# computational-cell-analytics/micro-sam

Measured on AMD Instinct MI355X. Metric: 1024^2 tiles/s embed+AMG (vit_b bf16), higher is better.
Workload: dtype bf16 image encoder (patch embedding + neck, 1.2 % of its flops, on hi+lo operand pairs of that type), fp16 mask decoder (16-bit MFMA operands, fp32 accumulation); 1 GPU; configs[1]: vit_b, 1024x1024 uint8 synthetic tiles, batched embedding precompute + AutomaticMaskGenerator (32x32 grid, multimask, default thresholds); encoder_batch=16, distinct_tiles_per_gpu=256, weights=seeded synthetic checkpoint (synthetic.py variant 'cells'), decode_lanes=3

## Files before the change

### include/msam_hip.h

```cpp
#ifndef MSAM_HIP_H
#define MSAM_HIP_H

#include <stdint.h>

#ifdef __cplusplus
extern "C" {
#endif

#define MSAM_MAX_BLOCKS 32
#define MSAM_F32 1
#define MSAM_BF16 2
#define MSAM_FP8 3
#define MSAM_F16 4
#define MSAM_U8 5
#define MSAM_U16 6
#define MSAM_ACT_NONE 0
#define MSAM_ACT_GELU 1
#define MSAM_ACT_RELU 2
#define MSAM_ACT_SIGMOID 3

const char* msam_last_error(void);
int msam_abi_version(void);


// ... 2 lines not shown
    const void* W; int64_t ldw;
    int32_t M, N, K;
    const float* bias;
    const float* table;
    int32_t table_rows, table_cols;
    int64_t table_ld;
    const void* resid;
    int32_t resid_dtype; int32_t resid_rows;
    int64_t ldr;
    int32_t act;
    void* out; int32_t out_dtype; int64_t ldc;
    int32_t out_mode;
    void* q; void* k; void* v;
    int32_t heads, head_dim, tokens;
    int32_t use_glds;
    int32_t ln_mode;
    const float* ln_w; const float* ln_b; float ln_eps;
    int32_t a_dtype;
    const float* row_scale; const float* col_scale;
    int32_t split_k;
    const float* ln_add; void* ln_out_a; void* ln_out_b;
} msam_gemm_t;
int msam_gemm_bf16(const msam_gemm_t* p, void* stream);
#define MSAM_GEMM_GROUP_MAX 5
int msam_gemm_group_bf16(const msam_gemm_t* items, int32_t n, void* stream);

typedef struct {
    const void* A; const void* W; int32_t M, N, K;
    const float* bias;
    const float* table; int32_t table_rows, table_cols; int64_t table_ld;
    const void* resid; int32_t resid_rows; int64_t ldr;
    int32_t ln_mode; const float* ln_w; const float* ln_b; float ln_eps;
    void* out; int64_t ldc;
    int32_t kv_split; void* k_out; void* vT_out; int32_t tokens;
    int32_t head_major;
} msam_wsgemm_t;
int msam_wsgemm_bf16(const msam_wsgemm_t* p, void* stream);

typedef struct {
    const void* xin; const void* q_shared;
    const void* wq; const float* bq; const float* peq;
    const void* wo; const float* bo; const float* ln_w; const float* ln_b; float ln_eps;
    const void* ktok; const void* vtok; int32_t Nt;
    void* out; int32_t rows;
} msam_image_layer_t;
int msam_decoder_image_layer(const msam_image_layer_t* p, void* stream);

int64_t msam_t2i_fold_workspace_bytes(int32_t P);
int msam_t2i_fold_attention(const void* keys, int32_t kv_shared, const void* qtok, int32_t P, int32_t Nt, const void* wk,
                            const void* tabk, const void* wv, const float* bv, void* out, void* workspace,
                            int64_t workspace_bytes, void* stream);

int64_t msam_i2t_fold_workspace_bytes(int32_t P);
int msam_i2t_fold_layer(const void* xin, int32_t x_shared, const void* ktok, const void* vtok, int32_t P, int32_t Nt,
                        const void* wq, const void* tabq, const void* wo, const float* bo, const float* ln_w,
                        const float* ln_b, float ln_eps, void* out, void* workspace, int64_t workspace_bytes, void* stream);

int64_t msam_chain_tables_bytes(void);
int msam_chain_prepare_tables(const void* src, const void* q0, const void* tabk, const void* tabq1, void* tables, void* stream);
int64_t msam_i2t_fold_operand_bytes(int32_t P);
int msam_i2t_fold_operands(const void* ktok, const void* vtok, int32_t P, int32_t Nt, const void* wq, const void* wo,
                           const float* bo, int32_t with_kfold, void* operands, void* stream);
int64_t msam_i2t0_t2i_workspace_bytes(int32_t P);
int msam_i2t0_t2i_fused(const void* tables, const void* operands0, const float* ln0_w, const float* ln0_b, float ln_eps,
                        const void* qtok, int32_t P, int32_t Nt, const void* wk, const void* wv, const float* bv, void* out,
                        void* workspace, int64_t workspace_bytes, void* stream);
int64_t msam_chain_tables2_bytes(void);
int msam_chain_prepare_tables2(const void* src, const void* wv, const float* bv, const void* wk, const float* ln0_w,
                               const float* ln0_b, const void* wo0, const float* bo0, void* tables2, void* stream);
int64_t msam_chain_const2_bytes(void);
int msam_chain_prepare_const2(const void* wv, const float* bv, const void* wk, const float* ln0_w, const float* ln0_b,
                              const void* wo0, const float* bo0, void* const2, void* stream);
int msam_chain_prepare_tables2_c(const void* src, const void* const2, void* tables2, void* stream);
int64_t msam_t2i_fold_values_bytes(int32_t P);
int msam_t2i_fold_values(const void* vtok0, int32_t P, int32_t Nt, const void* tables2, void* mf, void* stream);
int msam_i2t_fold_operands_values(const void* ktok, const void* vtok, int32_t P, int32_t Nt, const void* wq, const void* wo,
                                  const float* bo, int32_t with_kfold, const void* tables2, void* operands, void* mf, void* stream);
int64_t msam_i2t0_t2i_v2_workspace_bytes(int32_t P);
int msam_i2t0_t2i_fused_v2(const void* tables, const void* tables2, const void* operands0, const void* mf, const float* ln0_w,
                           float ln_eps, const void* qtok, int32_t P, int32_t Nt, const void* wk, void* out, void* workspace,
                           int64_t workspace_bytes, void* stream);
int msam_i2t01_fused(const void* tables, const void* operands0, const float* ln0_w, const float* ln0_b, const void* operands1,
                     const float* ln1_w, const float* ln1_b, float ln_eps, int32_t P, int32_t Nt, void* out, void* stream);

int msam_upscale_fused(const void* keys, int32_t P, const void* w1, const float* b1, const float* ln_w, const float* ln_b,
                       float ln_eps, const void* w2, const float* b2, const float* hyper, int32_t hyper_ld, int32_t mask0,
                       int32_t nmask, float* low_res, void* stream);
int msam_upscale_fused_layout(const void* keys, int32_t keys_blocked, int32_t P, const void* w1, const float* b1,
                              const float* ln_w, const float* ln_b, float ln_eps, const void* w2, const float* b2,
                              const float* hyper, int32_t hyper_ld, int32_t mask0, int32_t nmask, float* low_res, void* stream);
int msam_upscale_fused_out(const void* keys, int32_t keys_blocked, int32_t P, const void* w1, const float* b1,
                           const float* ln_w, const float* ln_b, float ln_eps, const void* w2, const float* b2,
                           const float* hyper, int32_t hyper_ld, int32_t mask0, int32_t nmask, void* low_res,
                           int32_t low_res_dtype, void* stream);

int msam_upscale_set_prio(int32_t prio);
int msam_fold_attn_set_dma(int32_t on);
int msam_tune_set(const char* key, int32_t value);
int msam_debug_i2t_timing(int32_t enable, uint64_t* host_out);
int msam_gemm256_set_staging(int staging);
int msam_gemm_set_trace(void* device_words);
int msam_profile_enable(int on);
int msam_profile_collect(int32_t* launches, double* total_ms, double* total_flops);
#define MSAM_PROFILE_FAMILIES 8
int msam_profile_collect_family(int32_t* launches, double* ms, double* flops, double* bytes);

int msam_to_image(const void* in, int32_t in_dtype, int32_t H, int32_t W, int32_t C, uint8_t* out, void* workspace, void* stream);

int msam_mask_nms(const uint32_t* bits, const int32_t* order, const float* boxes, const int32_t* area, int32_t K, int32_t H,
                  int32_t W, float thresh, int32_t intersection_over_min, uint64_t* mask_scratch, int32_t* keep_flags,
                  void* stream);

int64_t msam_amg_generate_workspace_bytes(int32_t N, int32_t H, int32_t W);
int msam_amg_generate_labels(const float* iou, const float* stability, const int32_t* boxes, const int32_t* area,
                             const uint32_t* bits, int32_t N, int32_t H, int32_t W, const int32_t* crop_box,
                             float pred_iou_thresh, float stability_score_thresh, float box_nms_thresh,
                             int32_t min_object_size, int32_t with_background, int32_t* labels, int32_t* flag,
                             void* workspace, int64_t workspace_bytes, void* stream);

int64_t msam_labels_from_masks_workspace_bytes(int32_t H, int32_t W);
int msam_labels_from_masks(const uint32_t* bits, const int32_t* order, int32_t K, const int32_t* k_dev, int32_t H, int32_t W,
                           int32_t min_object_size, int32_t with_background, int32_t* labels, int32_t* flag,
                           void* workspace, int64_t workspace_bytes, void* stream);

int msam_layernorm_backward(const float* x, const float* weight, const float* dy, float eps, int64_t rows, int32_t dim,
                            float* dx, float* dweight, float* dbias, void* stream);
int msam_attention_forward(const float* q, const float* k, const float* v, int32_t BH, int32_t Nq, int32_t Nk, int32_t D,
                           float scale, float* out, float* lse, void* stream);
int msam_attention_backward(const float* q, const float* k, const float* v, const float* out, const float* dout,
                            const float* lse, int32_t BH, int32_t Nq, int32_t Nk, int32_t D, float scale, float* dq, float* dk,
                            float* dv, float* delta, void* stream);

int msam_relpos_attention_forward(const float* q, const float* k, const float* v, const float* bias_h, const float* bias_w,
                                  int32_t BH, int32_t Gh, int32_t Gw, int32_t D, float scale, float* out, float* lse,
                                  void* stream);
int msam_relpos_attention_backward(const float* q, const float* k, const float* v, const float* bias_h, const float* bias_w,
                                   const float* out, const float* dout, const float* lse, int32_t BH, int32_t Gh, int32_t Gw,
                                   int32_t D, float scale, float* dq, float* dk, float* dv, float* dbias_h, float* dbias_w,
                                   float* delta, void* stream);

int msam_cast_transpose(const void* x, int32_t x_dtype, int64_t M, int32_t K, int64_t ldx, void* out16, void* outT, float* colsum,
                        void* stream);

int msam_layernorm(const float* x, const float* weight, const float* bias, float eps, int64_t rows, int32_t dim,
                   void* out, int32_t out_dtype, int32_t gelu, int32_t out_nchw_hw, void* stream);

int msam_layernorm_fp8(const float* x, const float* weight, const float* bias, float eps, int64_t rows, int32_t dim,
                       void* out_fp8, float* row_scale, void* stream);
int msam_quant_rows_fp8(const void* x_bf16, int64_t rows, int32_t dim, void* out_fp8, float* row_scale, void* stream);
int msam_patchify(const float* img, int32_t B, void* out_bf16, void* stream);
int msam_patchify16(const float* img, int32_t B, int32_t dtype16, void* out16, void* stream);
int msam_patchify_u8(const uint8_t* img, int32_t B, int32_t h, int32_t w, void* out_bf16, void* stream);
int msam_patchify_u8_16(const uint8_t* img, int32_t B, int32_t h, int32_t w, int32_t dtype16, void* out16, void* stream);
int msam_im2col3x3(const void* x_bf16, int32_t B, int32_t C, void* out_bf16, void* stream);
int msam_cast_f32_to_bf16(const float* x, void* out_bf16, int64_t n, void* stream);
int msam_cast_f32_to_16(const float* x, int32_t dtype16, void* out16, int64_t n, void* stream);
int msam_resample_u8(const uint8_t* in, int32_t B, int32_t H, int32_t W, int32_t C, int32_t axis, int32_t n_out,
                     const int32_t* bounds, const int32_t* coefs, int32_t ksize, uint8_t* out, void* stream);
int msam_patchify_split16(const float* img, int32_t B, int32_t dtype16, void* out16, void* stream);
int msam_patchify_u8_split16(const uint8_t* img, int32_t B, int32_t h, int32_t w, int32_t dtype16, void* out16, void* stream);
int msam_im2col3x3_split16(const float* x_f32, int32_t B, int32_t C, int32_t dtype16, void* out16, void* stream);
int msam_cast_f32_split16(const float* x, int32_t dtype16, void* out16, int64_t rows, int32_t dim, void* stream);

int msam_window_attention(const void* q, const void* k, const void* v, const void* rel_h, const void* rel_w,
                          const float* qkv_bias, int32_t B, int32_t heads, int32_t head_dim, float scale, void* out,
                          void* stream);
// ... 274 lines not shown
```

### micro_sam_amd/_lib.py

```python
from __future__ import annotations

import ctypes as C
import os
from typing import Optional

import torch

from . import build as _build

MSAM_MAX_BLOCKS = 32
F32, BF16, FP8, F16, U8, U16 = 1, 2, 3, 4, 5, 6
ACT_NONE, ACT_GELU, ACT_RELU, ACT_SIGMOID = 0, 1, 2, 3

_vp, _i32, _i64, _f32 = C.c_void_p, C.c_int32, C.c_int64, C.c_float
PROFILE_FAMILIES = 8


class GemmParams(C.Structure):
    _fields_ = [
        ("A", _vp), ("lda", _i64), ("W", _vp), ("ldw", _i64), ("M", _i32), ("N", _i32), ("K", _i32),
        ("bias", _vp), ("table", _vp), ("table_rows", _i32), ("table_cols", _i32), ("table_ld", _i64),
        ("resid", _vp), ("resid_dtype", _i32), ("resid_rows", _i32), ("ldr", _i64), ("act", _i32),
        ("out", _vp), ("out_dtype", _i32), ("ldc", _i64), ("out_mode", _i32),
        ("q", _vp), ("k", _vp), ("v", _vp), ("heads", _i32), ("head_dim", _i32), ("tokens", _i32),
# ... 63 lines not shown


class SGemmParams(C.Structure):
    _fields_ = [("A", _vp), ("lda", _i64), ("A2", _vp), ("lda2", _i64), ("a2_rows", _i64), ("W", _vp), ("ldw", _i64),
                ("M", _i64), ("N", _i32), ("K", _i32), ("bias", _vp), ("act", _i32), ("res", _vp), ("ldr", _i64), ("res_rows", _i64),
                ("out", _vp), ("ldc", _i64), ("col_scale", _vp), ("col_shift", _vp), ("conv_h", _i32), ("conv_w", _i32), ("conv_c", _i32),
                ("shuffle_h", _i32), ("shuffle_w", _i32), ("shuffle_c", _i32), ("a2_cols", _i32), ("split16", _i32), ("a_scale", _f32), ("w_scale", _f32), ("w_pairs", _vp)]


class SI2TParams(C.Structure):
    _fields_ = [("keys", _vp), ("key_batch_stride", _i64), ("pos", _vp), ("wq", _vp), ("bq", _vp), ("tok_k", _vp), ("tok_v", _vp),
                ("ld_tok", _i64), ("tok_batch_stride", _i64), ("wo", _vp), ("bo", _vp), ("ln_weight", _vp), ("ln_bias", _vp),
                ("ln_eps", _f32), ("denom", _f32), ("out", _vp), ("B", _i32), ("Tk", _i32), ("split16", _i32), ("wq_scale", _f32), ("wo_scale", _f32), ("wq_pairs", _vp), ("wo_pairs", _vp)]


class ST2IParams(C.Structure):
    _fields_ = [("keys", _vp), ("key_batch_stride", _i64), ("pos", _vp), ("q", _vp), ("ldq", _i64), ("wk", _vp), ("wv", _vp), ("bv", _vp),
                ("denom", _f32), ("out", _vp), ("ldo", _i64), ("B", _i32), ("Tk", _i32), ("workspace", _vp), ("workspace_bytes", _i64)]


class SUp2Params(C.Structure):
    _fields_ = [("u1", _vp), ("ln_weight", _vp), ("ln_bias", _vp), ("ln_eps", _f32), ("w2", _vp), ("b2", _vp), ("w_scale", _f32),
                ("hyper", _vp), ("hyper_ld", _i32), ("mask0", _i32), ("nmask", _i32), ("low_res", _vp), ("P", _i64)]


class MaskPromptParams(C.Structure):
    _fields_ = [(n, _vp) for n in ("c1_w", "c1_b", "ln1_w", "ln1_b", "c2_w", "c2_b", "ln2_w", "ln2_b", "c3_w", "c3_b")] + [("exact_gelu", _i32)]


_PROTOS = {
    "msam_last_error": (C.c_char_p, []),
    "msam_abi_version": (_i32, []),
    "msam_gemm_bf16": (_i32, [C.POINTER(GemmParams), _vp]),
    "msam_wsgemm_bf16": (_i32, [C.POINTER(WsGemmParams), _vp]),
    "msam_decoder_image_layer": (_i32, [C.POINTER(ImageLayerParams), _vp]),
    "msam_t2i_fold_workspace_bytes": (_i64, [_i32]),
    "msam_t2i_fold_attention": (_i32, [_vp, _i32, _vp, _i32, _i32, _vp, _vp, _vp, _vp, _vp, _vp, _i64, _vp]),
    "msam_upscale_fused": (_i32, [_vp, _i32, _vp, _vp, _vp, _vp, _f32, _vp, _vp, _vp, _i32, _i32, _i32, _vp, _vp]),
    "msam_uncrop_bits": (_i32, [_vp, _i32, _i32, _i32, _i32, _i32, _i32, _i32, _vp, _vp]),
    "msam_decoder_forward_masks": (_i32, [C.POINTER(DecoderParams), C.POINTER(MaskPromptParams), _vp, _vp, _vp, _vp, _i32, _vp, _vp,
                                          _i32, _i32, _vp, _vp, _vp, _i64, _vp]),
    "msam_i2t_fold_workspace_bytes": (_i64, [_i32]),
    "msam_i2t_fold_layer": (_i32, [_vp, _i32, _vp, _vp, _i32, _i32, _vp, _vp, _vp, _vp, _vp, _vp, _f32, _vp, _vp, _i64, _vp]),
    "msam_profile_enable": (_i32, [_i32]),
    "msam_profile_collect": (_i32, [C.POINTER(_i32), C.POINTER(C.c_double), C.POINTER(C.c_double)]),
    "msam_profile_collect_family": (_i32, [_i32 * PROFILE_FAMILIES, C.c_double * PROFILE_FAMILIES, C.c_double * PROFILE_FAMILIES,
                                          C.c_double * PROFILE_FAMILIES]),
    "msam_layernorm": (_i32, [_vp, _vp, _vp, _f32, _i64, _i32, _vp, _i32, _i32, _i32, _vp]),
    "msam_layernorm_backward": (_i32, [_vp, _vp, _vp, _f32, _i64, _i32, _vp, _vp, _vp, _vp]),
    "msam_attention_forward": (_i32, [_vp, _vp, _vp, _i32, _i32, _i32, _i32, _f32, _vp, _vp, _vp]),
    "msam_attention_backward": (_i32, [_vp, _vp, _vp, _vp, _vp, _vp, _i32, _i32, _i32, _i32, _f32, _vp, _vp, _vp, _vp, _vp]),
    "msam_relpos_attention_forward": (_i32, [_vp, _vp, _vp, _vp, _vp, _i32, _i32, _i32, _i32, _f32, _vp, _vp, _vp]),
    "msam_relpos_attention_backward": (_i32, [_vp, _vp, _vp, _vp, _vp, _vp, _vp, _vp, _i32, _i32, _i32, _i32, _f32, _vp, _vp, _vp,
                                              _vp, _vp, _vp, _vp]),
    "msam_amg_generate_workspace_bytes": (_i64, [_i32, _i32, _i32]),
    "msam_amg_generate_labels": (_i32, [_vp, _vp, _vp, _vp, _vp, _i32, _i32, _i32, C.POINTER(_i32), _f32, _f32, _f32, _i32, _i32,
                                        _vp, _vp, _vp, _i64, _vp]),
    "msam_to_image": (_i32, [_vp, _i32, _i32, _i32, _i32, _vp, _vp, _vp]),
    "msam_patchify": (_i32, [_vp, _i32, _vp, _vp]),
    "msam_patchify_u8": (_i32, [_vp, _i32, _i32, _i32, _vp, _vp]),
    "msam_im2col3x3": (_i32, [_vp, _i32, _i32, _vp, _vp]),
    "msam_cast_f32_to_bf16": (_i32, [_vp, _vp, _i64, _vp]),
    "msam_cast_transpose": (_i32, [_vp, _i32, _i64, _i32, _i64, _vp, _vp, _vp, _vp]),
    "msam_gemm256_set_staging": (_i32, [_i32]),
    "msam_gemm_set_trace": (_i32, [_vp]),
    "msam_gemm_group_bf16": (_i32, [_vp, _i32, _vp]),
    "msam_fold_attn_set_dma": (_i32, [_i32]),
    "msam_tune_set": (_i32, [C.c_char_p, _i32]),
    "msam_i2t_fold_operand_bytes": (_i64, [_i32]),
    "msam_i2t_fold_operands": (_i32, [_vp, _vp, _i32, _i32, _vp, _vp, _vp, _i32, _vp, _vp]),
    "msam_i2t0_t2i_workspace_bytes": (_i64, [_i32]),
    "msam_i2t0_t2i_fused": (_i32, [_vp, _vp, _vp, _vp, _f32, _vp, _i32, _i32, _vp, _vp, _vp, _vp, _vp, _i64, _vp]),
    "msam_i2t01_fused": (_i32, [_vp, _vp, _vp, _vp, _vp, _vp, _vp, _f32, _i32, _i32, _vp, _vp]),
    "msam_chain_tables2_bytes": (_i64, []),
    "msam_chain_prepare_tables2": (_i32, [_vp, _vp, _vp, _vp, _vp, _vp, _vp, _vp, _vp, _vp]),
    "msam_chain_const2_bytes": (_i64, []),
    "msam_chain_prepare_const2": (_i32, [_vp, _vp, _vp, _vp, _vp, _vp, _vp, _vp, _vp]),
    "msam_chain_prepare_tables2_c": (_i32, [_vp, _vp, _vp, _vp]),
    "msam_t2i_fold_values_bytes": (_i64, [_i32]),
    "msam_t2i_fold_values": (_i32, [_vp, _i32, _i32, _vp, _vp, _vp]),
    "msam_i2t_fold_operands_values": (_i32, [_vp, _vp, _i32, _i32, _vp, _vp, _vp, _i32, _vp, _vp, _vp, _vp]),
    "msam_i2t0_t2i_v2_workspace_bytes": (_i64, [_i32]),
    "msam_i2t0_t2i_fused_v2": (_i32, [_vp, _vp, _vp, _vp, _vp, _f32, _vp, _i32, _i32, _vp, _vp, _vp, _i64, _vp]),
    "msam_chain_tables_bytes": (_i64, []),
    "msam_chain_prepare_tables": (_i32, [_vp, _vp, _vp, _vp, _vp, _vp]),
    "msam_upscale_fused_layout": (_i32, [_vp, _i32, _i32, _vp, _vp, _vp, _vp, _f32, _vp, _vp, _vp, _i32, _i32, _i32, _vp, _vp]),
    "msam_upscale_fused_out": (_i32, [_vp, _i32, _i32, _vp, _vp, _vp, _vp, _f32, _vp, _vp, _vp, _i32, _i32, _i32, _vp, _i32, _vp]),
    "msam_upscale_set_prio": (_i32, [_i32]),
    "msam_layernorm_fp8": (_i32, [_vp, _vp, _vp, _f32, _i64, _i32, _vp, _vp, _vp]),
    "msam_quant_rows_fp8": (_i32, [_vp, _i64, _i32, _vp, _vp, _vp]),
    "msam_debug_i2t_timing": (_i32, [_i32, _vp]),
    "msam_window_attention": (_i32, [_vp, _vp, _vp, _vp, _vp, _vp, _i32, _i32, _i32, C.c_float, _vp, _vp]),
    "msam_global_attention": (_i32, [_vp, _vp, _vp, _vp, _vp, _i32, _i32, _i32, C.c_float, _vp, _vp]),
    "msam_window_attention16": (_i32, [_vp, _vp, _vp, _vp, _vp, _vp, _i32, _i32, _i32, C.c_float, _i32, _vp, _vp]),
    "msam_global_attention16": (_i32, [_vp, _vp, _vp, _vp, _vp, _i32, _i32, _i32, C.c_float, _i32, _vp, _vp]),
    "msam_patchify16": (_i32, [_vp, _i32, _i32, _vp, _vp]),
    "msam_patchify_u8_16": (_i32, [_vp, _i32, _i32, _i32, _i32, _vp, _vp]),
    "msam_cast_f32_to_16": (_i32, [_vp, _i32, _vp, _i64, _vp]),
    "msam_resample_u8": (_i32, [_vp, _i32, _i32, _i32, _i32, _i32, _i32, _vp, _vp, _i32, _vp, _vp]),
    "msam_patchify_split16": (_i32, [_vp, _i32, _i32, _vp, _vp]),
    "msam_patchify_u8_split16": (_i32, [_vp, _i32, _i32, _i32, _i32, _vp, _vp]),
    "msam_im2col3x3_split16": (_i32, [_vp, _i32, _i32, _i32, _vp, _vp]),
    "msam_cast_f32_split16": (_i32, [_vp, _i32, _vp, _i64, _i32, _vp]),
    "msam_encoder_workspace_bytes": (_i64, [C.POINTER(EncoderParams), _i32]),
    "msam_encoder_forward": (_i32, [C.POINTER(EncoderParams), _vp, _vp, _i32, _i32, _i32, _vp, _vp, _i64, _vp, _i32, _vp]),
    "msam_decoder_dtype": (_i32, []),
    "msam_decoder_const_bytes": (_i64, []),
    "msam_decoder_prepare_const": (_i32, [C.POINTER(DecoderParams), _vp, _vp]),
    "msam_decoder_image_bytes": (_i64, []),
    "msam_decoder_prepare_image": (_i32, [C.POINTER(DecoderParams), _vp, _vp, _vp, _vp, _i64, _vp]),
    "msam_decoder_workspace_bytes": (_i64, [_i32]),
    "msam_prompt_encode": (_i32, [C.POINTER(DecoderParams), C.POINTER(MaskPromptParams), _vp, _vp, _i32, _vp, _vp, _i32, _vp, _vp, _vp]),
    "msam_decoder_forward_embeddings": (_i32, [C.POINTER(DecoderParams), _vp, _vp, _vp, _i32, _vp, _vp, _i32, _i32, _vp, _vp, _vp,
                                               _i64, _vp]),
    "msam_decoder_forward": (_i32, [C.POINTER(DecoderParams), _vp, _vp, _vp, _vp, _i32, _vp, _i32, _i32, _vp, _vp, _vp,
                                    _i64, _vp]),
    "msam_postprocess_masks": (_i32, [_vp, _i32, _i32, _i32, _i32, _i32, _f32, _f32, _vp, _vp, _vp, _vp, _vp]),
    "msam_postprocess_masks16": (_i32, [_vp, _i32, _i32, _i32, _i32, _i32, _i32, _f32, _f32, _vp, _vp, _vp, _vp, _vp]),
    "msam_rle_run_counts": (_i32, [_vp, _i32, _i32, _i32, _vp, _vp]),
    "msam_rle_encode": (_i32, [_vp, _i32, _i32, _i32, _vp, _vp, _vp]),
    "msam_mask_nms": (_i32, [_vp, _vp, _vp, _vp, _i32, _i32, _i32, _f32, _i32, _vp, _vp, _vp]),
    "msam_box_nms": (_i32, [_vp, _i32, _f32, _vp, _vp, _vp]),
    "msam_box_nms_valid": (_i32, [_vp, _vp, _i32, _f32, _vp, _vp, _vp]),
    "msam_paint_label_image_dev": (_i32, [_vp, _vp, _vp, _i32, _i32, _vp, _vp]),
    "msam_label_components_async": (_i32, [_vp, _i32, _i32, _vp, _vp, _i32, _vp]),
    "msam_component_sizes": (_i32, [_vp, _i32, _vp, _vp, _vp]),
    "msam_labels_from_masks_workspace_bytes": (_i64, [_i32, _i32]),
    "msam_labels_from_masks": (_i32, [_vp, _vp, _i32, _vp, _i32, _i32, _i32, _i32, _vp, _vp, _vp, _i64, _vp]),
    "msam_host_seeded_watershed": (_i32, [_vp, _vp, _vp, _i32, _i32, _vp]),
    "msam_slice_overlaps": (_i32, [_vp, _i32, _i32, _i32, _vp, _vp, _i32, _vp, _i32, _vp, _vp]),
    "msam_paint_label_image": (_i32, [_vp, _vp, _i32, _i32, _i32, _vp, _vp]),
    "msam_label_components": (_i32, [_vp, _i32, _i32, _vp, _vp, _i32, C.POINTER(_i32), _vp]),
    "msam_strict_gemm": (_i32, [C.POINTER(SGemmParams), _vp]),
    "msam_strict_i2t_block": (_i32, [C.POINTER(SI2TParams), _vp]),
    "msam_strict_layernorm": (_i32, [_vp, _vp, _vp, _f32, _i64, _i32, _vp, _i32, _i32, _vp]),
    "msam_strict_relpos_attention": (_i32, [_vp, _vp, _vp, _vp, _i32, _i32, _i32, _i32, _i32, _f32, _vp, _vp]),
    "msam_split16_relpos_attention": (_i32, [_vp, _vp, _vp, _vp, _i32, _i32, _i32, _i32, _i32, _f32, _vp, _vp]),
    "msam_strict_attention": (_i32, [_vp, _i64, _i64, _vp, _i64, _i64, _vp, _i64, _i64, _i32, _i32, _i32, _i32, _i32, _f32, _vp, _i64,
                                     _i64, _vp]),
    "msam_strict_patchify": (_i32, [_vp, _vp, _i32, _i32, _i32, _vp, _vp]),
    "msam_strict_im2col3x3": (_i32, [_vp, _i32, _i32, _vp, _vp]),
    "msam_strict_source": (_i32, [_vp, _vp, _i64, _i32, _vp, _vp]),
    "msam_strict_hyper_masks": (_i32, [_vp, _vp, _i32, _i32, _i32, _i64, _vp, _vp]),
    "msam_strict_upscale2": (_i32, [C.POINTER(SUp2Params), _vp]),
    "msam_split16_t2i_attention": (_i32, [C.POINTER(ST2IParams), _vp]),
    "msam_split16_prepare_pairs": (_i32, [_vp, _i64, _i32, _f32, _i32, _vp, _vp]),
    "msam_split16_i2t_block": (_i32, [C.POINTER(SI2TParams), _vp, _i64, _vp]),
    "msam_strict_instance_norm": (_i32, [_vp, _i64, _i32, _i64, _i32, _f32, _vp, _vp, _i64, _vp]),
    "msam_strict_resize_bilinear": (_i32, [_vp, _i32, _i32, _i32, _i32, _i32, _i64, _i32, _i32, _i32, _f32, _f32, _i32, _vp, _vp]),
    "msam_objfeat_gather": (_i32, [_vp, _vp, _i32, _i32, _vp, _vp, _i32, _vp, _vp, _vp]),
    "msam_objfeat_accumulate": (_i32, [_vp, _vp, _i32, _vp, _vp, _vp, _vp, _vp, _vp, _vp, _i32, _i32, _i32, _vp, _vp]),
    "msam_objfeat_finish": (_i32, [_vp, _vp, _vp, _i32, _vp, _vp, _i32, _vp, _vp]),
    "msam_objfeat_project": (_i32, [_vp, _i64, _vp, _i32, _vp, _vp]),
    "msam_label_matching_workspace_bytes": (_i64, [_i32, _i32]),
    "msam_label_matching": (_i32, [_vp, _vp, _i32, _i32, _i32, _i32, C.POINTER(C.c_double), _i32, _vp, _i64, _i32, _vp, _i32, _vp]),
    "msam_edt_squared_workspace_bytes": (_i64, [_i32, _i32]),
    "msam_edt_squared": (_i32, [_vp, _i32, _i32, _i32, _vp, _vp, _i64, _vp]),
    "msam_label_props_workspace_bytes": (_i64, [_i32, _i32, _i32]),
    "msam_label_props": (_i32, [_vp, _i32, _i32, _vp, _i32, _vp, _vp, _vp, _vp, _vp, _i64, _vp]),
    "msam_distance_targets_workspace_bytes": (_i64, [_i32, _i32, _i32]),
    "msam_distance_targets": (_i32, [_vp, _i32, _i32, _i32, _i32, _f32, _vp, _vp, _vp, _vp, _vp, _i64, _vp]),
    "msam_mask_pack": (_i32, [_vp, _i32, _i32, _i32, _vp, _vp]),
    "msam_mask_iou_counts": (_i32, [_vp, _vp, _i32, _i32, _i32, C.c_double, _vp, _vp, _vp]),
    "msam_mask_box_prompts": (_i32, [_vp, _i32, _i32, _i32, C.c_double, _i32, _i32, _vp, _vp, _vp]),
    "msam_mask_logits": (_i32, [_vp, _i32, _i32, _i32, _vp, _vp]),
    "msam_paint_max": (_i32, [_vp, _vp, _vp, _i32, _i32, _i32, _vp, _vp]),
# ... 78 lines not shown
```

### micro_sam_amd/csrc/decfold.hip

```cpp
#include "common.h"
#include "../../include/msam_hip.h"
#include <string>

void msam_set_error(const char* msg);
int msam_check_launch(const char* what);
void msam_profile_mark2(void* stream, int begin, double flops, double bytes, int family);

namespace {

constexpr int T = 4096, C = 256, CI = 128, TK = 32, NTHR = 256;
constexpr int SUBT = 1024 + 32;
constexpr int KEYS_BYTES = 16 * SUBT, TAB_BYTES = TK * CI * 2, BUF_BYTES = KEYS_BYTES + TAB_BYTES;
constexpr float NEG_BIG = -1.0e30f;
#ifndef FOLD_ATTN_DMA_DEFAULT
#define FOLD_ATTN_DMA_DEFAULT 0
#endif

typedef short s16x4_t __attribute__((ext_vector_type(4)));

MSAM_DEVINL uint2 lds_tr16(const unsigned char* p) {
    s16x4_t v = __builtin_amdgcn_ds_read_tr16_b64_v4i16((s16x4_t __attribute__((address_space(3)))*)p);
    return __builtin_bit_cast(uint2, v);
}

// ... 594 lines not shown
    const double bytes = (double)((kv_shared & 1) ? 1 : P) * T * C * 2 + (KS > 1 ? (double)P * KS * 64 * C * 4 : 0.0);
    msam_profile_mark2(stream, 1, flops, bytes, 3);
    if (g_fold_attn_dma && !a.blocked) {
        const int grid3 = a.nitems < 3 * cus ? a.nitems : 3 * cus;
        hipLaunchKernelGGL(fold_attn_kernel<true>, dim3(grid3), dim3(NTHR), 0, s, a);
    } else {
        hipLaunchKernelGGL(fold_attn_kernel<false>, dim3(grid), dim3(NTHR), 0, s, a);
    }
    msam_profile_mark2(stream, 0, flops, bytes, 3);
    if (int e = msam_check_launch("fold_attn")) return e;
    if (KS == 1) return 0;
    hipLaunchKernelGGL(fold_finish_kernel, dim3(P * 8), dim3(128), 0, s, opart, stats, KS, Nt, (const u16*)wv, bv, (u16*)out);
    return msam_check_launch("fold_finish");
}

int64_t msam_i2t_tok_workspace_bytes(int32_t P);
int msam_i2t_tok_layer(const void* xin, int32_t x_shared, const void* ktok, const void* vtok, int32_t P, int32_t Nt,
                       const void* wq, const void* tabq, const void* wo, const float* bo, const float* ln_w,
                       const float* ln_b, float ln_eps, void* out, void* workspace, int KS, void* stream);
extern int g_tune_i2t_variant;

extern "C" int64_t msam_i2t_fold_workspace_bytes(int32_t P) {
    const int64_t a = (int64_t)P * 64 * C * 2 * 2, b = msam_i2t_tok_workspace_bytes(P);
    return a > b ? a : b;
}

extern "C" int msam_i2t_fold_layer(const void* xin, int32_t x_shared, const void* ktok, const void* vtok, int32_t P,
                                   int32_t Nt, const void* wq, const void* tabq, const void* wo, const float* bo,
                                   const float* ln_w, const float* ln_b, float ln_eps, void* out, void* workspace,
                                   int64_t workspace_bytes, void* stream) {
    if (!xin || !ktok || !vtok || !wq || !tabq || !wo || !bo || !ln_w || !ln_b || !out || !workspace || P <= 0) {
        msam_set_error("msam_i2t_fold_layer: null argument");
        return 1;
    }
    if (Nt < 1 || Nt > 8) { msam_set_error("msam_i2t_fold_layer: 1 <= Nt <= 8 tokens per prompt"); return 1; }
    if (workspace_bytes < msam_i2t_fold_workspace_bytes(P)) { msam_set_error("msam_i2t_fold_layer: workspace too small"); return 1; }
    if (g_tune_i2t_variant == 1)
        return msam_i2t_tok_layer(xin, x_shared, ktok, vtok, P, Nt, wq, tabq, wo, bo, ln_w, ln_b, ln_eps, out, workspace,
                                  key_splits(P), stream);
    hipStream_t s = (hipStream_t)stream;
    u16* kfold = (u16*)workspace;
    u16* vfoldT = kfold + (long)P * 64 * C;
    hipLaunchKernelGGL(fold_q_kernel, dim3(P * 8), dim3(256), 0, s, (const u16*)ktok, (const u16*)wq, Nt, kfold);
    if (int e = msam_check_launch("fold_k")) return e;
    hipLaunchKernelGGL(fold_v_kernel, dim3(P), dim3(256), 0, s, (const u16*)vtok, (const u16*)wo, Nt, vfoldT);
    if (int e = msam_check_launch("fold_v")) return e;
    I2tArgs a{};
    a.xin = (const u16*)xin; a.x_shared = x_shared; a.kfold = kfold; a.vfoldT = vfoldT; a.ktok = (const u16*)ktok; a.Nt = Nt;
    a.tabq = (const u16*)tabq; a.bo = bo; a.ln_w = ln_w; a.ln_b = ln_b; a.eps = ln_eps;
    a.KS = key_splits(P); a.nitems = P * a.KS; a.out = (u16*)out;
    int dev = 0, cus = 256;
    (void)hipGetDevice(&dev);
    (void)hipDeviceGetAttribute(&cus, hipDeviceAttributeMultiprocessorCount, dev);
    const int grid = a.nitems < 2 * cus ? a.nitems : 2 * cus;
    const double flops = (double)P * T * (2.0 * 64 * C * 2 + 2.0 * 64 * 32);
    const double bytes = (double)(x_shared ? 1 : P) * T * C * 2 + (double)P * T * C * 2;
    msam_profile_mark2(stream, 1, flops, bytes, 2);
    if (g_i2t_timing) hipLaunchKernelGGL(fold_i2t_kernel<true>, dim3(grid), dim3(NTHR), 0, s, a);
    else hipLaunchKernelGGL(fold_i2t_kernel<false>, dim3(grid), dim3(NTHR), 0, s, a);
    msam_profile_mark2(stream, 0, flops, bytes, 2);
    return msam_check_launch("fold_i2t");
}

extern "C" int msam_debug_i2t_timing(int32_t enable, uint64_t* host_out) {
    g_i2t_timing = enable;
    if (host_out) {
        if (hipDeviceSynchronize() != hipSuccess ||
            hipMemcpyFromSymbol(host_out, HIP_SYMBOL(g_i2t_stamps), sizeof(unsigned long long) * 64 * 12) != hipSuccess) {
            msam_set_error("msam_debug_i2t_timing: copy failed");
            return 2;
        }
    }
    return 0;
}

extern "C" int msam_fold_attn_set_dma(int32_t on) { g_fold_attn_dma = on; return 0; }

extern int g_tune_i2t_wg_per_cu, g_tune_chain_variant, g_tune_chain_tmask, g_tune_up_gelu16, g_tune_up_ln_two_pass, g_tune_up_centred;
void msam_gemm_set_dbg(int v);
void msam_gemm_set_gw(int delay, int cls);
void msam_gemm_set_g3(int delay);
void msam_gemm_set_g3_epi(int v);
extern int g_tune_tok_fuse;
extern int g_tune_mlp_split_fused;
extern int g_tune_sgemm_bufs, g_tune_srel_mfma, g_tune_sgemm_small_below, g_tune_si2t_dbg, g_tune_si2t_late_us, g_tune_sattn_allh;
int g_tune_dec_chain = 1, g_tune_dec_chain_min_p = 128;
extern "C" int msam_tune_set(const char* key, int32_t value) {
    const std::string k = key ? key : "";
    if (k == "i2t_variant") g_tune_i2t_variant = value;
    else if (k == "i2t_wg_per_cu") g_tune_i2t_wg_per_cu = value;
    else if (k == "dec_chain") g_tune_dec_chain = value;
    else if (k == "chain_variant") g_tune_chain_variant = value;
    else if (k == "chain_tmask") g_tune_chain_tmask = value;
    else if (k == "up_gelu16") g_tune_up_gelu16 = value;
    else if (k == "up_ln_two_pass") g_tune_up_ln_two_pass = value;
    else if (k == "up_centred") g_tune_up_centred = value;
    else if (k == "gemm_dbg") msam_gemm_set_dbg(value);
    else if (k == "gw_delay") msam_gemm_set_gw(value, -1);
    else if (k == "gw_class") msam_gemm_set_gw(-2, value);
    else if (k == "g3_delay") msam_gemm_set_g3(value);
    else if (k == "g3_epi") msam_gemm_set_g3_epi(value);
    else if (k == "tok_fuse") g_tune_tok_fuse = value;
    else if (k == "mlp_split_fused") g_tune_mlp_split_fused = value;
    else if (k == "dec_chain_min_p") g_tune_dec_chain_min_p = value;
    else if (k == "sgemm_bufs") g_tune_sgemm_bufs = value;
    else if (k == "srel_mfma") g_tune_srel_mfma = value;
    else if (k == "sattn_allh") g_tune_sattn_allh = value;
    else if (k == "sgemm_small_below") g_tune_sgemm_small_below = value;
    else if (k == "si2t_dbg") g_tune_si2t_dbg = value;
    else if (k == "si2t_late_us") g_tune_si2t_late_us = value;
    else { msam_set_error("msam_tune_set: unknown key"); return 1; }
    return 0;
}
```

### micro_sam_amd/csrc/decfold_tok.hip

```cpp
#include "common.h"
#include "../../include/msam_hip.h"

void msam_set_error(const char* msg);
int msam_check_launch(const char* what);
void msam_profile_mark2(void* stream, int begin, double flops, double bytes, int family);

int g_tune_i2t_variant = 1;
int g_tune_i2t_wg_per_cu = 2;
int g_tune_chain_tmask = 255;
int g_tune_chain_variant = 9;

namespace {

constexpr int T = 4096, C = 256, CI = 128, NTHR = 256;
constexpr int FRAG = 1024;
constexpr int KT_OFF = 0, KT_BYTES = 4 * 2 * FRAG;
constexpr int KF_OFF = KT_OFF + KT_BYTES, KF_BYTES = 4 * 8 * FRAG;
constexpr int VF_OFF = KF_OFF + KF_BYTES, VF_BYTES = 2 * 16 * FRAG;
constexpr int OPER_BYTES = VF_OFF + VF_BYTES;
constexpr float NEG_BIG = -1.0e30f;
constexpr float SCALE = 0.25f * 1.4426950408889634f;

__global__ __launch_bounds__(256) void fold_frag_kernel(const u16* __restrict__ ktok, const u16* __restrict__ vtok,
                                                        const u16* __restrict__ wq, const u16* __restrict__ wo,
                                                        const float* __restrict__ bo, int Nt, int with_kf,
                                                        u16* __restrict__ oper, const unsigned char* __restrict__ t2 = nullptr,
                                                        u16* __restrict__ mf = nullptr) {
    __shared__ __attribute__((aligned(16))) u16 img[OPER_BYTES / 2];
    __shared__ float kk[8][CI], vv[8][CI];
    const int p = blockIdx.x, c = threadIdx.x;
    for (int i = c; i < 8 * CI; i += 256) {
        const int t = i >> 7, d = i & (CI - 1);
        kk[t][d] = t < Nt ? d2f(ktok[((long)p * Nt + t) * CI + d]) : 0.f;
        vv[t][d] = t < Nt ? d2f(vtok[((long)p * Nt + t) * CI + d]) : 0.f;
    }
    for (int i = c; i < KT_BYTES / 16; i += 256) ((uint4*)img)[KT_OFF / 16 + i] = make_uint4(0, 0, 0, 0);
    __syncthreads();
    if (with_kf) {
        const int ks = c >> 5, fg = (c >> 3) & 3, ii = c & 7;
        for (int h = 0; h < 8; ++h) {
            float w[16];
#pragma unroll
            for (int d = 0; d < 16; ++d) w[d] = d2f(wq[(h * 16 + d) * C + c]);
#pragma unroll
            for (int t = 0; t < 8; ++t) {
                float acc = 0.f;
#pragma unroll
                for (int d = 0; d < 16; ++d) acc = fmaf(kk[t][h * 16 + d], w[d], acc);
                const int m = 2 * (h >> 2) + (t >> 2), fr = 4 * (h & 3) + (t & 3);
                img[KF_OFF / 2 + ((m * 8 + ks) * 64 + fg * 16 + fr) * 8 + ii] = f2d(acc * SCALE);
            }
        }
    }
    for (int j = c; j < 8 * 8 * 16; j += 256) {
        const int h = j >> 7, t = (j >> 4) & 7, d = j & 15;
        const int m = 2 * (h >> 2) + (t >> 2), e = (h >> 1) & 1, fr = 4 * (h & 3) + (t & 3), fg = 2 * (h & 1) + (d >> 3);
        img[KT_OFF / 2 + ((m * 2 + e) * 64 + fg * 16 + fr) * 8 + (d & 7)] = f2d(kk[t][h * 16 + d] * SCALE);
    }
    {
        const int cp = c >> 5, within = c & 31, rho = 4 * (within >> 3) + (within & 3), ct = 2 * cp + ((within >> 2) & 1);
        const float bo8 = bo[c] * 0.125f;
        for (int h = 0; h < 8; ++h) {
            const uint4 w0 = *(const uint4*)(wo + (long)c * CI + h * 16), w1 = *(const uint4*)(wo + (long)c * CI + h * 16 + 8);
            const uint32_t ww[8] = {w0.x, w0.y, w0.z, w0.w, w1.x, w1.y, w1.z, w1.w};
            float wf[16];
#pragma unroll
            for (int x = 0; x < 8; ++x) { wf[2 * x] = d2f((u16)(ww[x] & 0xffff)); wf[2 * x + 1] = d2f((u16)(ww[x] >> 16)); }
            uint32_t pk[4];
#pragma unroll
            for (int t2 = 0; t2 < 4; ++t2) {
                float a0 = 0.f, a1 = 0.f;
#pragma unroll
                for (int d = 0; d < 16; ++d) { a0 = fmaf(wf[d], vv[2 * t2][h * 16 + d], a0); a1 = fmaf(wf[d], vv[2 * t2 + 1][h * 16 + d], a1); }
                pk[t2] = pack2d(2 * t2 < Nt ? a0 + bo8 : 0.f, 2 * t2 + 1 < Nt ? a1 + bo8 : 0.f);
            }
            const int a = h >> 2, fg = h & 3;
            *(uint4*)(img + VF_OFF / 2 + ((a * 16 + ct) * 64 + fg * 16 + rho) * 8) = make_uint4(pk[0], pk[1], pk[2], pk[3]);
        }
    }
    if (t2) {
        const int d = c & 127, hh = c >> 7;
        const float* wowv = (const float*)t2 + d * 128;
        const float cd8 = ((const float*)(t2 + 128 * 128 * 4))[d] * 0.125f;
        u16* mdst = mf + (long)p * (16 * FRAG / 2);
        for (int h = hh * 4; h < hh * 4 + 4; ++h) {
            float wv_[16];
#pragma unroll
            for (int e = 0; e < 16; ++e) wv_[e] = wowv[h * 16 + e];
            uint32_t pk[4];
#pragma unroll
            for (int t2_ = 0; t2_ < 4; ++t2_) {
                float a0 = 0.f, a1 = 0.f;
#pragma unroll
// ... 93 lines not shown
    const float nmr = -mean * rstd;
#pragma unroll
    for (int c2 = 0; c2 < 8; ++c2) {
        const float4 g0 = *(const float4*)(gp + c2 * 32), g1 = *(const float4*)(gp + c2 * 32 + 4);
        const float4 h0 = *(const float4*)(gp + C + c2 * 32), h1 = *(const float4*)(gp + C + c2 * 32 + 4);
        const f32x4_t x0 = o[2 * c2], x1 = o[2 * c2 + 1];
        y[c2].x = pack2d(fmaf(fmaf(x0[0], rstd, nmr), g0.x, h0.x), fmaf(fmaf(x0[1], rstd, nmr), g0.y, h0.y));
        y[c2].y = pack2d(fmaf(fmaf(x0[2], rstd, nmr), g0.z, h0.z), fmaf(fmaf(x0[3], rstd, nmr), g0.w, h0.w));
        y[c2].z = pack2d(fmaf(fmaf(x1[0], rstd, nmr), g1.x, h1.x), fmaf(fmaf(x1[1], rstd, nmr), g1.y, h1.y));
        y[c2].w = pack2d(fmaf(fmaf(x1[2], rstd, nmr), g1.z, h1.z), fmaf(fmaf(x1[3], rstd, nmr), g1.w, h1.w));
    }
}

struct TokArgs {
    const u16* xin; int x_shared;
    const u16* oper;
    const u16* tabq;
    const float* ln_w; const float* ln_b; float eps;
    int Nt, nitems, KS;
    u16* out;
};

__global__ __launch_bounds__(NTHR, 2) void i2t_tok_kernel(TokArgs a) {
    __shared__ __attribute__((aligned(16))) unsigned char lds[OPER_BYTES + 2 * C * 4];
    const int tid = threadIdx.x, lane = tid & 63, w = __builtin_amdgcn_readfirstlane(tid >> 6), fr = lane & 15, fg = lane >> 4;
    const int ks_sh = __builtin_ctz(a.KS), tpi_sh = 8 - ks_sh;
    const int TPI = 1 << tpi_sh, nt = TPI >> 2;
    float* prm = (float*)(lds + OPER_BYTES);
    prm[tid] = a.ln_w[tid]; prm[C + tid] = a.ln_b[tid];
    const WaveConst wc = wave_const(fr, fg, a.Nt);
    const int voff = fr * (C * 2) + fg * 16;
    const int tvoff = fr * (CI * 2) + fg * 16;
    const rsrc_t rtab = make_rsrc(a.tabq, T * CI * 2);
    const unsigned char* const L = lds + lane * 16;
    const float* const gp = prm + fg * 8;

    for (int item = (int)blockIdx.x; item < a.nitems; item += (int)gridDim.x) {
        const int p = __builtin_amdgcn_readfirstlane(item >> ks_sh), split = __builtin_amdgcn_readfirstlane(item & (a.KS - 1));
        __syncthreads();
        {
            const uint4* src = (const uint4*)(a.oper + (long)p * (OPER_BYTES / 2));
#pragma unroll 6
            for (int i = tid; i < OPER_BYTES / 16; i += NTHR) ((uint4*)lds)[i] = src[i];
        }
        __syncthreads();
        const rsrc_t rx = make_rsrc(a.xin + (long)(a.x_shared ? 0 : p) * T * C, T * C * 2);
        const rsrc_t ro = make_rsrc(a.out + (long)p * T * C, T * C * 2);
        const int tile0 = split * TPI + w;

        uint4 b[8], tb[4];
#define TK_LOAD(tile_)                                                                             \
        do {                                                                                       \
            const int so_ = (tile_) * (16 * C * 2), to_ = (tile_) * (16 * CI * 2);                 \
            _Pragma("unroll") for (int s_ = 0; s_ < 8; ++s_) b[s_] = buf_load16(rx, voff, so_ + s_ * 64);      \
            _Pragma("unroll") for (int s_ = 0; s_ < 4; ++s_) tb[s_] = buf_load16(rtab, tvoff, to_ + s_ * 64);  \
        } while (0)
        TK_LOAD(tile0);
        wait_vmem_all();
        for (int n = 0; n < nt; ++n) {
            asm volatile("" ::: "memory");
            const int tile = tile0 + 4 * n;
            uint4 y[8];
            i2t_block<KT_OFF, KF_OFF, VF_OFF, true>(L, gp, a.eps, b, tb, wc, y, [&]() {
                const int nx = tile0 + 4 * (n + 1 < nt ? n + 1 : nt - 1);
                TK_LOAD(nx);
            });
#pragma unroll
            for (int c2 = 0; c2 < 8; ++c2) buf_store16(y[c2], ro, voff, tile * (16 * C * 2) + c2 * 64);
        }
#undef TK_LOAD
    }
}

struct ChainArgs {
    const u16* src;
    const u16* q0;
    const u16* oper0;
    const float* ln0_w; const float* ln0_b;
    const u16* oper1;
    const u16* tabq1;
    const float* ln1_w; const float* ln1_b;
    float eps; int Nt, P;
    u16* out;
};

constexpr int NTHR8 = 512;
constexpr int C_KT0 = 0, C_VF0 = C_KT0 + KT_BYTES, C_KT1 = C_VF0 + VF_BYTES, C_KF1 = C_KT1 + KT_BYTES, C_VF1 = C_KF1 + KF_BYTES,
              C_PRM = C_VF1 + VF_BYTES, C_LDS = C_PRM + 4 * C * 4;

__global__ __launch_bounds__(NTHR8, 2) void i2t01_kernel(ChainArgs a) {
    __shared__ __attribute__((aligned(16))) unsigned char lds[C_LDS];
    const int tid = threadIdx.x, lane = tid & 63, w = __builtin_amdgcn_readfirstlane(tid >> 6), fr = lane & 15, fg = lane >> 4;
    float* prm = (float*)(lds + C_PRM);
    if (tid < C) { prm[tid] = a.ln0_w[tid]; prm[C + tid] = a.ln0_b[tid]; }
    else { prm[2 * C + tid - C] = a.ln1_w[tid - C]; prm[3 * C + tid - C] = a.ln1_b[tid - C]; }
    const WaveConst wc = wave_const(fr, fg, a.Nt);
    const int voff = lane * 16, tvoff = lane * 16;
    const rsrc_t rsrc = make_rsrc(a.src, T * C * 2), rq0 = make_rsrc(a.q0, T * CI * 2), rtab = make_rsrc(a.tabq1, T * CI * 2);
    const unsigned char* const L = lds + lane * 16;
    const float* const gp0 = prm + fg * 8;
    const float* const gp1 = prm + 2 * C + fg * 8;
    constexpr int NT = 256 / 8;

    for (int p = (int)blockIdx.x; p < a.P; p += (int)gridDim.x) {
        __syncthreads();
        {
            const uint4* s0 = (const uint4*)(a.oper0 + (long)p * (OPER_BYTES / 2));
            const uint4* s1 = (const uint4*)(a.oper1 + (long)p * (OPER_BYTES / 2));
            for (int i = tid; i < KT_BYTES / 16; i += NTHR8) ((uint4*)(lds + C_KT0))[i] = s0[KT_OFF / 16 + i];
            for (int i = tid; i < VF_BYTES / 16; i += NTHR8) ((uint4*)(lds + C_VF0))[i] = s0[VF_OFF / 16 + i];
#pragma unroll 3
            for (int i = tid; i < OPER_BYTES / 16; i += NTHR8) ((uint4*)(lds + C_KT1))[i] = s1[i];
        }
        __syncthreads();
        const rsrc_t ro = make_rsrc(a.out + (long)p * T * C, T * C * 2);
        uint4 b[8], qi[4], tb[4];
#define CH_LOAD0(tile_)                                                                            \
        do {                                                                                       \
            const int so_ = (tile_) * (16 * C * 2), to_ = (tile_) * (16 * CI * 2);                 \
            _Pragma("unroll") for (int s_ = 0; s_ < 8; ++s_) b[s_] = buf_load16(rsrc, voff, so_ + s_ * FRAG);    \
            _Pragma("unroll") for (int s_ = 0; s_ < 4; ++s_) qi[s_] = buf_load16(rq0, tvoff, to_ + s_ * FRAG);   \
        } while (0)
#define CH_LOAD1(tile_)                                                                            \
        do {                                                                                       \
            const int to_ = (tile_) * (16 * CI * 2);                                               \
            _Pragma("unroll") for (int s_ = 0; s_ < 4; ++s_) tb[s_] = buf_load16(rtab, tvoff, to_ + s_ * FRAG);  \
        } while (0)
        CH_LOAD0(w); CH_LOAD1(w);
        wait_vmem_all();
        for (int n = 0; n < NT; ++n) {
            asm volatile("" ::: "memory");
            const int tile = w + 8 * n, nx = w + 8 * (n + 1 < NT ? n + 1 : NT - 1);
            uint4 y1[8], y2[8];
            i2t_block<C_KT0, 0, C_VF0, false>(L, gp0, a.eps, b, qi, wc, y1, [&]() { CH_LOAD0(nx); });
            i2t_block<C_KT1, C_KF1, C_VF1, true>(L, gp1, a.eps, y1, tb, wc, y2, [&]() { CH_LOAD1(nx); });
#pragma unroll
            for (int c2 = 0; c2 < 8; ++c2) buf_store16(y2[c2], ro, voff, tile * (16 * C * 2) + c2 * FRAG);
        }
#undef CH_LOAD0
#undef CH_LOAD1
    }
}

struct AttnState { f32x4_t o[8]; float m[4], l[4]; };

template <int QD, int QF, int WV, class F>
MSAM_DEVINL void t2i_block(const unsigned char* L, const uint4* y, const uint4* tk, AttnState& st, F&& consumed) {
    f32x4_t s[4];
    uint4 fa[4], fb[4];
#pragma unroll
    for (int ct = 0; ct < 4; ++ct) s[ct] = f32x4_t{0.f, 0.f, 0.f, 0.f};
    TK_RD4(fa, QF, 8 * FRAG);
    TK_FENCE();
#pragma unroll
    for (int g = 0; g < 9; ++g) {
        uint4* cur = (g & 1) ? fb : fa;
        uint4* nxt = (g & 1) ? fa : fb;
        if (g + 1 < 8) TK_RD4(nxt, QF + (g + 1) * FRAG, 8 * FRAG);
        else if (g + 1 < 9) TK_RD4(nxt, QD, FRAG);
        else TK_RD4(nxt, WV, 8 * FRAG);
#pragma unroll
        for (int ct = 0; ct < 4; ++ct) s[ct] = mfma16d(g < 8 ? y[g < 8 ? g : 0] : tk[ct], cur[ct], s[ct]);
        TK_FENCE();
    }
    consumed();
    float mloc[4];
    bool need = false;
// ... 72 lines not shown
    float* prm = (float*)(lds + F_PRM);
    if (tid < C) prm[tid] = a.ln0_w[tid]; else prm[tid] = a.ln0_b[tid - C];
    for (int i = tid; i < WV_BYTES / 16; i += NTHR8) ((uint4*)(lds + F_WV))[i] = ((const uint4*)a.wvfrag)[i];
    const WaveConst wc = wave_const(fr, fg, a.Nt);
    const int voff = lane * 16, tvoff = lane * 16;
    const rsrc_t rsrc = make_rsrc(a.src, T * C * 2), rq0 = make_rsrc(a.q0, T * CI * 2), rtab = make_rsrc(a.tabk, T * CI * 2);
    const unsigned char* const L = lds + lane * 16;
    const float* const gp0 = prm + fg * 8;
    constexpr int NT = 256 / 8;

    for (int p = (int)blockIdx.x; p < a.P; p += (int)gridDim.x) {
        __syncthreads();
        {
            const uint4* s0 = (const uint4*)(a.oper0 + (long)p * (OPER_BYTES / 2));
            const uint4* s1 = (const uint4*)(a.aoper + (long)p * (AOPER_BYTES / 2));
            for (int i = tid; i < KT_BYTES / 16; i += NTHR8) ((uint4*)(lds + F_KT0))[i] = s0[KT_OFF / 16 + i];
            for (int i = tid; i < VF_BYTES / 16; i += NTHR8) ((uint4*)(lds + F_VF0))[i] = s0[VF_OFF / 16 + i];
            for (int i = tid; i < AOPER_BYTES / 16; i += NTHR8) ((uint4*)(lds + F_QD))[i] = s1[i];
        }
        __syncthreads();
        AttnState st;
#pragma unroll
        for (int h = 0; h < 8; ++h) st.o[h] = f32x4_t{0.f, 0.f, 0.f, 0.f};
#pragma unroll
        for (int ct = 0; ct < 4; ++ct) { st.m[ct] = NEG_BIG; st.l[ct] = 0.f; }
        uint4 b[8], qi[4], tk[4];
#define FU_LOAD0(tile_)                                                                            \
        do {                                                                                       \
            const int so_ = (tile_) * (16 * C * 2), to_ = (tile_) * (16 * CI * 2);                 \
            _Pragma("unroll") for (int s_ = 0; s_ < 8; ++s_) b[s_] = buf_load16(rsrc, voff, so_ + s_ * FRAG);    \
            _Pragma("unroll") for (int s_ = 0; s_ < 4; ++s_) qi[s_] = buf_load16(rq0, tvoff, to_ + s_ * FRAG);   \
        } while (0)
#define FU_LOAD1(tile_)                                                                            \
        do {                                                                                       \
            const int to_ = (tile_) * (16 * CI * 2);                                               \
            _Pragma("unroll") for (int s_ = 0; s_ < 4; ++s_) tk[s_] = buf_load16(rtab, tvoff, to_ + s_ * FRAG);  \
        } while (0)
        FU_LOAD0(w); FU_LOAD1(w);
        for (int n = 0; n < NT; ++n) {
            asm volatile("" ::: "memory");
            const int nx = w + 8 * (n + 1 < NT ? n + 1 : NT - 1);
            uint4 y1[8];
            i2t_block<F_KT0, 0, F_VF0, false>(L, gp0, a.eps, b, qi, wc, y1, [&]() { FU_LOAD0(nx); });
            t2i_block<F_QD, F_QF, F_WV>(L, y1, tk, st, [&]() { FU_LOAD1(nx); });
        }
#undef FU_LOAD0
#undef FU_LOAD1
#pragma unroll
        for (int ct = 0; ct < 4; ++ct) { st.l[ct] += __shfl_xor(st.l[ct], 16); st.l[ct] += __shfl_xor(st.l[ct], 32); }
        __syncthreads();
        float* mg = (float*)lds + w * MERGE_FLOATS;
        if (fg == 0) {
#pragma unroll
            for (int ct = 0; ct < 4; ++ct) { mg[ct * 16 + fr] = st.m[ct]; mg[64 + ct * 16 + fr] = st.l[ct]; }
        }
#pragma unroll
        for (int h = 0; h < 8; ++h)
            if ((fr >> 3) == (h & 1))
                *(float4*)(mg + 128 + (h * 8 + (fr & 7)) * 16 + fg * 4) = make_float4(st.o[h][0], st.o[h][1], st.o[h][2], st.o[h][3]);
        __syncthreads();
        {
            const int col = tid >> 3, d0 = (tid & 7) * 2, h = col >> 3, t = col & 7;
            const float* g0 = (const float*)lds;
            float mx = NEG_BIG;
#pragma unroll
            for (int ww = 0; ww < 8; ++ww) mx = fmaxf(mx, g0[ww * MERGE_FLOATS + col]);
            float lt = 0.f, o0 = 0.f, o1 = 0.f;
#pragma unroll
            for (int ww = 0; ww < 8; ++ww) {
                const float* gw = g0 + ww * MERGE_FLOATS;
                const float sc = __builtin_amdgcn_exp2f(gw[col] - mx);
                lt = fmaf(sc, gw[64 + col], lt);
                o0 = fmaf(sc, gw[128 + col * 16 + d0], o0); o1 = fmaf(sc, gw[128 + col * 16 + d0 + 1], o1);
            }
            if (t < a.Nt) {
                const float inv = 1.f / lt;
                *(uint32_t*)(a.out + ((long)p * a.Nt + t) * CI + h * 16 + d0) =
                    pack2d(fmaf(o0, inv, a.bv[h * 16 + d0]), fmaf(o1, inv, a.bv[h * 16 + d0 + 1]));
            }
        }
    }
}

template <int G, int D = 2> struct Ring { uint4 buf[D][G]; };

template <int G, class Off, int ABL = 0>
MSAM_DEVINL void ring_fill(Ring<G, Off::D>& r, const unsigned char* L, int batch) {
    if (ABL & 32) return;
#pragma unroll
    for (int j = 0; j < G; ++j) r.buf[batch % Off::D][j] = *(const uint4*)(L + Off::off((batch * G + j) % Off::N));
}
#define RING_STEP(n_) do { if ((n_) % G == 0) { TK_FENCE(); ring_fill<G, Off, ABL>(ring, L, (n_) / G + Off::D - 1); TK_FENCE(); } } while (0)
#define RING_AT(n_) ring.buf[((n_) / G) % Off::D][(n_) % G]

template <int G, class Off, int BASE, bool HAS_KF, int ABL = 0, bool AFFINE = true, class F>
MSAM_DEVINL void i2t_block_r(Ring<G, Off::D>& ring, const unsigned char* L, const float* gp, float eps, const uint4* b, const uint4* tb,
                             const WaveConst& wc, uint4* y, F&& consumed, uint4* pk_out = nullptr, float* stat_out = nullptr) {
    constexpr int NS = HAS_KF ? 40 : 8, G0 = HAS_KF ? 0 : 8;
    f32x4_t s[4];
#pragma unroll
    for (int m = 0; m < 4; ++m) s[m] = wc.sinit[m & 1];
#pragma unroll
    for (int i = 0; i < NS; ++i) {
        const int n = BASE + i, g = G0 + i / 4, m = i % 4;
        RING_STEP(n);
        if (!(ABL & 1)) s[m] = mfma16d(RING_AT(n), g < 8 ? b[g < 8 ? g : 0] : tb[2 * (m >> 1) + (g < 8 ? 0 : g - 8)], s[m]);
        else if (i < 4) s[m][0] += __uint_as_float((RING_AT(n).x ^ tb[m].x) & 0x3fffffffu);
    }
    f32x4_t o[16];
#pragma unroll
    for (int ct = 0; ct < 16; ++ct) o[ct] = mfma16d(wc.sel[ct & 1], b[ct >> 1], f32x4_t{0.f, 0.f, 0.f, 0.f});
    consumed();
    uint4 pk[2];
#pragma unroll
    for (int a2 = 0; a2 < 2; ++a2) {
        const f32x4_t u = s[2 * a2], v = s[2 * a2 + 1];
        const float mx = fmaxf(fmaxf(fmaxf(u[0], u[1]), fmaxf(u[2], u[3])), fmaxf(fmaxf(v[0], v[1]), fmaxf(v[2], v[3])));
        float eu[4], ev[4];
#pragma unroll
        for (int r = 0; r < 4; ++r) {
            eu[r] = (ABL & 64) ? u[r] - mx : __builtin_amdgcn_exp2f(u[r] - mx); ev[r] = (ABL & 64) ? v[r] - mx : __builtin_amdgcn_exp2f(v[r] - mx);
        }
        const float l = ((eu[0] + eu[1]) + (eu[2] + eu[3])) + ((ev[0] + ev[1]) + (ev[2] + ev[3]));
        const float inv = __builtin_amdgcn_rcpf(l);
        pk[a2] = make_uint4(pack2d(eu[0] * inv, eu[1] * inv), pack2d(eu[2] * inv, eu[3] * inv),
                            pack2d(ev[0] * inv, ev[1] * inv), pack2d(ev[2] * inv, ev[3] * inv));
    }
#pragma unroll
    for (int i = 0; i < 32; ++i) {
        const int n = BASE + NS + i;
        RING_STEP(n);
        if (!(ABL & 2) || i % 16 == 0) o[i % 16] = mfma16d(RING_AT(n), pk[i / 16], o[i % 16]);
    }
    if (ABL & 4) {
#pragma unroll
        for (int c2 = 0; c2 < 8; ++c2)
            y[c2] = make_uint4(pack2d(o[2 * c2][0], o[2 * c2][1]), pack2d(o[2 * c2][2], o[2 * c2][3]),
                               pack2d(o[2 * c2 + 1][0], o[2 * c2 + 1][1]), pack2d(o[2 * c2 + 1][2], o[2 * c2 + 1][3]));
        return;
    }
    float s1 = 0.f, s2 = 0.f;
#pragma unroll
    for (int ct = 0; ct < 16; ++ct)
#pragma unroll
        for (int r = 0; r < 4; ++r) { s1 += o[ct][r]; s2 = fmaf(o[ct][r], o[ct][r], s2); }
    s1 += __shfl_xor(s1, 16); s2 += __shfl_xor(s2, 16);
    s1 += __shfl_xor(s1, 32); s2 += __shfl_xor(s2, 32);
    const float mean = s1 * (1.f / C);
    const float rstd = rsqrtf(fmaxf(s2 * (1.f / C) - mean * mean, 0.f) + eps);
    const float nmr = -mean * rstd;
    if (pk_out) { pk_out[0] = pk[0]; pk_out[1] = pk[1]; }
    if (stat_out) { stat_out[0] = rstd; stat_out[1] = nmr; }
    if (!AFFINE) {
#pragma unroll
        for (int c2 = 0; c2 < 8; ++c2) {
            const f32x4_t x0 = o[2 * c2], x1 = o[2 * c2 + 1];
            y[c2] = make_uint4(pack2d(fmaf(x0[0], rstd, nmr), fmaf(x0[1], rstd, nmr)), pack2d(fmaf(x0[2], rstd, nmr), fmaf(x0[3], rstd, nmr)),
                               pack2d(fmaf(x1[0], rstd, nmr), fmaf(x1[1], rstd, nmr)), pack2d(fmaf(x1[2], rstd, nmr), fmaf(x1[3], rstd, nmr)));
        }
        return;
    }
#pragma unroll
    for (int c2 = 0; c2 < 8; ++c2) {
        const float4 g0 = *(const float4*)(gp + c2 * 32), g1 = *(const float4*)(gp + c2 * 32 + 4);
        const float4 h0 = *(const float4*)(gp + C + c2 * 32), h1 = *(const float4*)(gp + C + c2 * 32 + 4);
        const f32x4_t x0 = o[2 * c2], x1 = o[2 * c2 + 1];
        y[c2].x = pack2d(fmaf(fmaf(x0[0], rstd, nmr), g0.x, h0.x), fmaf(fmaf(x0[1], rstd, nmr), g0.y, h0.y));
        y[c2].y = pack2d(fmaf(fmaf(x0[2], rstd, nmr), g0.z, h0.z), fmaf(fmaf(x0[3], rstd, nmr), g0.w, h0.w));
        y[c2].z = pack2d(fmaf(fmaf(x1[0], rstd, nmr), g1.x, h1.x), fmaf(fmaf(x1[1], rstd, nmr), g1.y, h1.y));
        y[c2].w = pack2d(fmaf(fmaf(x1[2], rstd, nmr), g1.z, h1.z), fmaf(fmaf(x1[3], rstd, nmr), g1.w, h1.w));
    }
}

template <int G, class Off, int BASE, int ABL = 0, bool COMPACT = false, class F>
MSAM_DEVINL void t2i_block_r(Ring<G, Off::D>& ring, const unsigned char* L, const uint4* y, const uint4* tk, AttnState& st, F&& consumed) {
    f32x4_t s[4];
#pragma unroll
    for (int ct = 0; ct < 4; ++ct) s[ct] = f32x4_t{0.f, 0.f, 0.f, 0.f};
#pragma unroll
    for (int i = 0; i < 36; ++i) {
        const int n = BASE + i, g = i / 4, ct = i % 4;
        RING_STEP(n);
        if (!(ABL & 8)) s[ct] = mfma16d(g < 8 ? y[g < 8 ? g : 0] : tk[ct], RING_AT(n), s[ct]);
        else if (i < 4) s[ct][0] += __uint_as_float((RING_AT(n).x ^ tk[ct].x ^ y[ct].x ^ y[4 + ct].y) & 0x3fffffffu);
    }
    consumed();
    float mloc[4];
    bool need = false;
#pragma unroll
    for (int ct = 0; ct < 4; ++ct) {
        mloc[ct] = fmaxf(fmaxf(s[ct][0], s[ct][1]), fmaxf(s[ct][2], s[ct][3]));
        need = need || (mloc[ct] > st.m[ct] + 8.f);
    }
    if (__builtin_amdgcn_ballot_w64(need) != 0) {
#pragma unroll
        for (int ct = 0; ct < 4; ++ct) {
            float mx = mloc[ct];
            mx = fmaxf(mx, __shfl_xor(mx, 16)); mx = fmaxf(mx, __shfl_xor(mx, 32));
            const float mn = fmaxf(st.m[ct], mx), alpha = __builtin_amdgcn_exp2f(st.m[ct] - mn);
            st.m[ct] = mn; st.l[ct] *= alpha;
#pragma unroll
            for (int r = 0; r < 4; ++r) {
                if (COMPACT) st.o[ct][r] *= alpha;
                else { st.o[2 * ct][r] *= alpha; st.o[2 * ct + 1][r] *= alpha; }
            }
        }
    }
    uint4 pb[4];
#pragma unroll
    for (int ct = 0; ct < 4; ++ct) {
        float e[4];
#pragma unroll
        for (int r = 0; r < 4; ++r) e[r] = (ABL & 64) ? s[ct][r] - st.m[ct] : __builtin_amdgcn_exp2f(s[ct][r] - st.m[ct]);
        st.l[ct] += (e[0] + e[1]) + (e[2] + e[3]);
        pb[ct] = make_uint4(pack2d(e[0], e[1]), pack2d(e[2], e[3]), 0u, 0u);
    }
    f32x4_t v[8];
#pragma unroll
    for (int h = 0; h < 8; ++h) v[h] = f32x4_t{0.f, 0.f, 0.f, 0.f};
#pragma unroll
    for (int i = 0; i < 64; ++i) {
        const int n = BASE + 36 + i, ks = i / 8, h = i % 8;
        RING_STEP(n);
        if (!(ABL & 16) || ks == 0) v[h] = mfma16d(y[(ABL & 16) ? h : ks], RING_AT(n), v[h]);
    }
    const bool hi_cols = (__lane_id() & 8) != 0;
#pragma unroll
    for (int h = 0; h < 8; ++h) {
        const uint4 va = make_uint4(pack2d(v[h][0], v[h][1]), pack2d(v[h][2], v[h][3]), 0u, 0u);
        if (COMPACT) {
            const bool mine = hi_cols == ((h & 1) != 0);
            const uint4 pm = make_uint4(mine ? pb[h >> 1].x : 0u, mine ? pb[h >> 1].y : 0u, 0u, 0u);
            st.o[h >> 1] = mfma16d(va, pm, st.o[h >> 1]);
        } else {
            st.o[h] = mfma16d(va, pb[h >> 1], st.o[h]);
        }
    }
}

template <int G, int D_ = 2> struct ChainOff {
    static constexpr int D = D_, USED = 112, N = ((USED + D * G - 1) / (D * G)) * (D * G);
    static __device__ constexpr int off(int n) {
        if (n < 8) return C_KT0 + ((n % 4) * 2 + n / 4) * FRAG;
        if (n < 40) return C_VF0 + (n - 8) * FRAG;
        if (n < 80) { const int i = n - 40, g = i / 4, m = i % 4; return g < 8 ? C_KF1 + (m * 8 + g) * FRAG : C_KT1 + (m * 2 + (g - 8)) * FRAG; }
        if (n < 112) return C_VF1 + (n - 80) * FRAG;
        return C_KT0;
    }
};
template <int G, int D_ = 2> struct FuseOff {
    static constexpr int D = D_, USED = 140, N = ((USED + D * G - 1) / (D * G)) * (D * G);
    static __device__ constexpr int off(int n) {
        if (n < 8) return F_KT0 + ((n % 4) * 2 + n / 4) * FRAG;
        if (n < 40) return F_VF0 + (n - 8) * FRAG;
        if (n < 76) { const int i = n - 40, g = i / 4, ct = i % 4; return g < 8 ? F_QF + (ct * 8 + g) * FRAG : F_QD + ct * FRAG; }
        if (n < 140) { const int i = n - 76, ks = i / 8, h = i % 8; return F_WV + (h * 8 + ks) * FRAG; }
        return F_KT0;
    }
};

template <int NW, int G, int D = 2, bool LATE = false>
__global__ __launch_bounds__(64 * NW, NW == 4 ? 1 : 2) void i2t01_ring_kernel(ChainArgs a) {
    typedef ChainOff<G, D> Off;
    constexpr int ABL = 0;
    constexpr int NTH = 64 * NW, NT = 256 / NW;
    __shared__ __attribute__((aligned(16))) unsigned char lds[C_LDS];
    const int tid = threadIdx.x, lane = tid & 63, w = __builtin_amdgcn_readfirstlane(tid >> 6), fr = lane & 15, fg = lane >> 4;
    float* prm = (float*)(lds + C_PRM);
    for (int i = tid; i < 4 * C; i += NTH) prm[i] = i < C ? a.ln0_w[i] : i < 2 * C ? a.ln0_b[i - C] : i < 3 * C ? a.ln1_w[i - 2 * C] : a.ln1_b[i - 3 * C];
    const WaveConst wc = wave_const(fr, fg, a.Nt);
    const int voff = lane * 16, tvoff = lane * 16;
    const rsrc_t rsrc = make_rsrc(a.src, T * C * 2), rq0 = make_rsrc(a.q0, T * CI * 2), rtab = make_rsrc(a.tabq1, T * CI * 2);
    const unsigned char* const L = lds + lane * 16;
    const float* const gp0 = prm + fg * 8;
    const float* const gp1 = prm + 2 * C + fg * 8;
    Ring<G, D> ring;
    for (int p = (int)blockIdx.x; p < a.P; p += (int)gridDim.x) {
        __syncthreads();
        {
            const uint4* s0 = (const uint4*)(a.oper0 + (long)p * (OPER_BYTES / 2));
            const uint4* s1 = (const uint4*)(a.oper1 + (long)p * (OPER_BYTES / 2));
            for (int i = tid; i < KT_BYTES / 16; i += NTH) ((uint4*)(lds + C_KT0))[i] = s0[KT_OFF / 16 + i];
            for (int i = tid; i < VF_BYTES / 16; i += NTH) ((uint4*)(lds + C_VF0))[i] = s0[VF_OFF / 16 + i];
#pragma unroll 3
            for (int i = tid; i < OPER_BYTES / 16; i += NTH) ((uint4*)(lds + C_KT1))[i] = s1[i];
        }
        __syncthreads();
        const rsrc_t ro = make_rsrc(a.out + (long)p * T * C, T * C * 2);
        uint4 b[8], qi[4], tb[4];
#define CH_LOAD0(tile_)                                                                            \
        do {                                                                                       \
            const int so_ = (tile_) * (16 * C * 2), to_ = (tile_) * (16 * CI * 2);                 \
            _Pragma("unroll") for (int s_ = 0; s_ < 8; ++s_) b[s_] = buf_load16(rsrc, voff, so_ + s_ * FRAG);    \
            _Pragma("unroll") for (int s_ = 0; s_ < 4; ++s_) qi[s_] = buf_load16(rq0, tvoff, to_ + s_ * FRAG);   \
        } while (0)
#define CH_LOAD1(tile_)                                                                            \
        do {                                                                                       \
            const int to_ = (tile_) * (16 * CI * 2);                                               \
            _Pragma("unroll") for (int s_ = 0; s_ < 4; ++s_) tb[s_] = buf_load16(rtab, tvoff, to_ + s_ * FRAG);  \
        } while (0)
        CH_LOAD0(w);
        if (!LATE) CH_LOAD1(w);
        wait_vmem_all();
#pragma unroll
        for (int k = 0; k + 1 < D; ++k) ring_fill<G, Off>(ring, L, k);
        for (int n = 0; n < NT; ++n) {
            asm volatile("" ::: "memory");
            const int tile = w + NW * n, nx = w + NW * (n + 1 < NT ? n + 1 : NT - 1);
            uint4 y1[8], y2[8];
            i2t_block_r<G, Off, 0, false>(ring, L, gp0, a.eps, b, qi, wc, y1, [&]() { if (LATE) CH_LOAD1(tile); else CH_LOAD0(nx); });
            i2t_block_r<G, Off, 40, true>(ring, L, gp1, a.eps, y1, tb, wc, y2, [&]() { if (LATE) CH_LOAD0(nx); else CH_LOAD1(nx); });
#pragma unroll
            for (int i = Off::USED; i < Off::N; ++i) RING_STEP(i);
#pragma unroll
            for (int c2 = 0; c2 < 8; ++c2) buf_store16(y2[c2], ro, voff, tile * (16 * C * 2) + c2 * FRAG);
        }
#undef CH_LOAD0
#undef CH_LOAD1
    }
}

template <int NW, int G, int ABL = 0, int D = 2, bool COMPACT = false, bool LATE = false>
__global__ __launch_bounds__(64 * NW, NW == 4 ? 1 : 2) void i2t0_t2i_ring_kernel(FuseArgs a) {
    typedef FuseOff<G, D> Off;
    constexpr int NTH = 64 * NW, NT = 256 / NW;
    __shared__ __attribute__((aligned(16))) unsigned char lds[F_LDS];
    const int tid = threadIdx.x, lane = tid & 63, w = __builtin_amdgcn_readfirstlane(tid >> 6), fr = lane & 15, fg = lane >> 4;
    float* prm = (float*)(lds + F_PRM);
    for (int i = tid; i < 2 * C; i += NTH) prm[i] = i < C ? a.ln0_w[i] : a.ln0_b[i - C];
    for (int i = tid; i < WV_BYTES / 16; i += NTH) ((uint4*)(lds + F_WV))[i] = ((const uint4*)a.wvfrag)[i];
    const WaveConst wc = wave_const(fr, fg, a.Nt);
    const int voff = lane * 16, tvoff = lane * 16;
    const rsrc_t rsrc = make_rsrc(a.src, T * C * 2), rq0 = make_rsrc(a.q0, T * CI * 2), rtab = make_rsrc(a.tabk, T * CI * 2);
    const unsigned char* const L = lds + lane * 16;
    const float* const gp0 = prm + fg * 8;
    Ring<G, D> ring;
    for (int p = (int)blockIdx.x; p < a.P; p += (int)gridDim.x) {
        __syncthreads();
        {
            const uint4* s0 = (const uint4*)(a.oper0 + (long)p * (OPER_BYTES / 2));
            const uint4* s1 = (const uint4*)(a.aoper + (long)p * (AOPER_BYTES / 2));
            for (int i = tid; i < KT_BYTES / 16; i += NTH) ((uint4*)(lds + F_KT0))[i] = s0[KT_OFF / 16 + i];
            for (int i = tid; i < VF_BYTES / 16; i += NTH) ((uint4*)(lds + F_VF0))[i] = s0[VF_OFF / 16 + i];
            for (int i = tid; i < AOPER_BYTES / 16; i += NTH) ((uint4*)(lds + F_QD))[i] = s1[i];
        }
        __syncthreads();
        AttnState st;
#pragma unroll
        for (int h = 0; h < 8; ++h) st.o[h] = f32x4_t{0.f, 0.f, 0.f, 0.f};
#pragma unroll
        for (int ct = 0; ct < 4; ++ct) { st.m[ct] = NEG_BIG; st.l[ct] = 0.f; }
        uint4 b[8], qi[4], tk[4];
#define FU_LOAD0(tile_)                                                                            \
        do {                                                                                       \
            const int so_ = (tile_) * (16 * C * 2), to_ = (tile_) * (16 * CI * 2);                 \
            _Pragma("unroll") for (int s_ = 0; s_ < 8; ++s_) b[s_] = buf_load16(rsrc, voff, so_ + s_ * FRAG);    \
            _Pragma("unroll") for (int s_ = 0; s_ < 4; ++s_) qi[s_] = buf_load16(rq0, tvoff, to_ + s_ * FRAG);   \
        } while (0)
#define FU_LOAD1(tile_)                                                                            \
        do {                                                                                       \
            const int to_ = (tile_) * (16 * CI * 2);                                               \
            _Pragma("unroll") for (int s_ = 0; s_ < 4; ++s_) tk[s_] = buf_load16(rtab, tvoff, to_ + s_ * FRAG);  \
        } while (0)
        FU_LOAD0(w & a.tmask);
        if (!LATE) FU_LOAD1(w & a.tmask);
        if (ABL & 32) {
#pragma unroll
            for (int j = 0; j < G; ++j)
#pragma unroll
                for (int k = 0; k < D; ++k) ring.buf[k][j] = make_uint4(tid, lane, 0x3c003c00u, 0x3c003c00u);
        }
#pragma unroll
        for (int k = 0; k + 1 < D; ++k) ring_fill<G, Off, ABL>(ring, L, k);
        for (int n = 0; n < NT; ++n) {
            asm volatile("" ::: "memory");
            const int nx = (w + NW * (n + 1 < NT ? n + 1 : NT - 1)) & a.tmask, cur = (w + NW * n) & a.tmask;
            uint4 y1[8];
            i2t_block_r<G, Off, 0, false, ABL>(ring, L, gp0, a.eps, b, qi, wc, y1, [&]() { if (LATE) FU_LOAD1(cur); else FU_LOAD0(nx); });
            t2i_block_r<G, Off, 40, ABL, COMPACT>(ring, L, y1, tk, st, [&]() { if (LATE) FU_LOAD0(nx); else FU_LOAD1(nx); });
#pragma unroll
            for (int i = Off::USED; i < Off::N; ++i) RING_STEP(i);
        }
#undef FU_LOAD0
#undef FU_LOAD1
#pragma unroll
        for (int ct = 0; ct < 4; ++ct) { st.l[ct] += __shfl_xor(st.l[ct], 16); st.l[ct] += __shfl_xor(st.l[ct], 32); }
        __syncthreads();
        float* mg = (float*)lds + w * MERGE_FLOATS;
        if (fg == 0) {
#pragma unroll
            for (int ct = 0; ct < 4; ++ct) { mg[ct * 16 + fr] = st.m[ct]; mg[64 + ct * 16 + fr] = st.l[ct]; }
        }
        if (COMPACT) {
#pragma unroll
            for (int ct = 0; ct < 4; ++ct)
                *(float4*)(mg + 128 + (ct * 16 + fr) * 16 + fg * 4) = make_float4(st.o[ct][0], st.o[ct][1], st.o[ct][2], st.o[ct][3]);
        } else {
#pragma unroll
            for (int h = 0; h < 8; ++h)
                if ((fr >> 3) == (h & 1))
                    *(float4*)(mg + 128 + (h * 8 + (fr & 7)) * 16 + fg * 4) = make_float4(st.o[h][0], st.o[h][1], st.o[h][2], st.o[h][3]);
        }
        __syncthreads();
        for (int idx = tid; idx < 512; idx += NTH) {
            const int col = idx >> 3, d0 = (idx & 7) * 2, h = col >> 3, t = col & 7;
            const float* g0 = (const float*)lds;
            float mx = NEG_BIG;
#pragma unroll
            for (int ww = 0; ww < NW; ++ww) mx = fmaxf(mx, g0[ww * MERGE_FLOATS + col]);
            float lt = 0.f, o0 = 0.f, o1 = 0.f;
#pragma unroll
            for (int ww = 0; ww < NW; ++ww) {
                const float* gw = g0 + ww * MERGE_FLOATS;
                const float sc = __builtin_amdgcn_exp2f(gw[col] - mx);
                lt = fmaf(sc, gw[64 + col], lt);
                o0 = fmaf(sc, gw[128 + col * 16 + d0], o0); o1 = fmaf(sc, gw[128 + col * 16 + d0 + 1], o1);
            }
            if (t < a.Nt) {
                const float inv = 1.f / lt;
                *(uint32_t*)(a.out + ((long)p * a.Nt + t) * CI + h * 16 + d0) =
                    pack2d(fmaf(o0, inv, a.bv[h * 16 + d0]), fmaf(o1, inv, a.bv[h * 16 + d0 + 1]));
            }
        }
    }
}

struct AttnOff2 {
    static constexpr int KT0 = 0, VF0 = KT0 + KT_BYTES, QD2 = VF0 + VF_BYTES, QF2 = QD2 + 4 * FRAG, MF2 = QF2 + 32 * FRAG,
                         COLC = MF2 + 16 * FRAG, GDT = COLC + 64 * 4, LDS = GDT + 128 * 4;
};
constexpr int AOPER2_BYTES = 4 * FRAG + 32 * FRAG;
constexpr int AOPER2_STRIDE = AOPER2_BYTES + 256;
constexpr int MF_BYTES = 16 * FRAG;
constexpr long T2_WOWV = 0, T2_CD = 128 * 128 * 4, T2_GD = T2_CD + 512, T2_BWV = T2_GD + 512, T2_KB = T2_BWV + 512,
               T2_TABV = T2_KB + 512, T2_WVG = T2_TABV + (long)T * CI * 2 ,
               T2_TABV_RM = T2_WVG + (long)CI * C * 2 , T2_BYTES = T2_TABV_RM + (long)T * CI * 2;

template <int G, int D_ = 2> struct FuseOff2 {
    static constexpr int D = D_, USED = 92, N = ((USED + D * G - 1) / (D * G)) * (D * G);
    static __device__ constexpr int off(int n) {
        if (n < 8) return AttnOff2::KT0 + ((n % 4) * 2 + n / 4) * FRAG;
        if (n < 40) return AttnOff2::VF0 + (n - 8) * FRAG;
        if (n < 76) { const int i = n - 40, g = i / 4, ct = i % 4; return g < 8 ? AttnOff2::QF2 + (ct * 8 + g) * FRAG : AttnOff2::QD2 + ct * FRAG; }
        if (n < 92) { const int i = n - 76, dv = i / 2, a2 = i % 2; return AttnOff2::MF2 + (a2 * 8 + dv) * FRAG; }
        return AttnOff2::KT0;
    }
};

struct FuseArgs2 {
    const u16* src; const u16* q0; const u16* tabk;
    const u16* tabv; const float* gd; const float* bwv;
    const u16* oper0;
    const u16* aoper;
    const u16* mf;
    float eps; int Nt, P;
    u16* out;
};

template <int G, class Off, int BASE, class F0, class F>
MSAM_DEVINL void t2i_block_v2(Ring<G, Off::D>& ring, const unsigned char* L, const uint4* y, const uint4* tk, const uint4* tv,
                              const uint4* pk0, float rstd, float nmr, const float* colc, const float* gd, AttnState& st, F0&& start,
                              F&& consumed) {
    constexpr int ABL = 0;
    start();
    f32x4_t s[4];
#pragma unroll
    for (int ct = 0; ct < 4; ++ct) { const float c_ = colc[ct * 16]; s[ct] = f32x4_t{c_, c_, c_, c_}; }
#pragma unroll
    for (int i = 0; i < 36; ++i) {
        const int n = BASE + i, g = i / 4, ct = i % 4;
        RING_STEP(n);
        s[ct] = mfma16d(g < 8 ? y[g < 8 ? g : 0] : tk[ct], RING_AT(n), s[ct]);
    }
    consumed();
    float mloc[4];
    bool need = false;
#pragma unroll
    for (int ct = 0; ct < 4; ++ct) {
        mloc[ct] = fmaxf(fmaxf(s[ct][0], s[ct][1]), fmaxf(s[ct][2], s[ct][3]));
        need = need || (mloc[ct] > st.m[ct] + 8.f);
    }
    if (__builtin_amdgcn_ballot_w64(need) != 0) {
#pragma unroll
        for (int ct = 0; ct < 4; ++ct) {
            float mx = mloc[ct];
            mx = fmaxf(mx, __shfl_xor(mx, 16)); mx = fmaxf(mx, __shfl_xor(mx, 32));
            const float mn = fmaxf(st.m[ct], mx), alpha = __builtin_amdgcn_exp2f(st.m[ct] - mn);
            st.m[ct] = mn; st.l[ct] *= alpha;
#pragma unroll
            for (int r = 0; r < 4; ++r) { st.o[2 * ct][r] *= alpha; st.o[2 * ct + 1][r] *= alpha; }
        }
    }
    uint4 pb[4];
#pragma unroll
    for (int ct = 0; ct < 4; ++ct) {
        float e[4];
#pragma unroll
        for (int r = 0; r < 4; ++r) e[r] = __builtin_amdgcn_exp2f(s[ct][r] - st.m[ct]);
        st.l[ct] += (e[0] + e[1]) + (e[2] + e[3]);
        pb[ct] = make_uint4(pack2d(e[0], e[1]), pack2d(e[2], e[3]), 0u, 0u);
    }
    float rr[4], nn[4];
    const int row0 = (__lane_id() >> 4) * 4;
#pragma unroll
    for (int r = 0; r < 4; ++r) { rr[r] = __shfl(rstd, row0 + r); nn[r] = __shfl(nmr, row0 + r); }
    const uint32_t* tvw = (const uint32_t*)tv;
#pragma unroll
    for (int dv = 0; dv < 8; ++dv) {
        f32x4_t v = {0.f, 0.f, 0.f, 0.f};
#pragma unroll
        for (int a2 = 0; a2 < 2; ++a2) {
            const int n = BASE + 36 + dv * 2 + a2;
            RING_STEP(n);
            v = mfma16d(pk0[a2], RING_AT(n), v);
        }
        const uint32_t w0 = tvw[2 * dv], w1 = tvw[2 * dv + 1];
        const float t0 = d2f((u16)(w0 & 0xffff)), t1 = d2f((u16)(w0 >> 16)), t2 = d2f((u16)(w1 & 0xffff)), t3 = d2f((u16)(w1 >> 16));
        const float g = gd[dv * 16];
        const float v0 = fmaf(rr[0], v[0] + t0, nn[0] * g), v1 = fmaf(rr[1], v[1] + t1, nn[1] * g);
        const float v2 = fmaf(rr[2], v[2] + t2, nn[2] * g), v3 = fmaf(rr[3], v[3] + t3, nn[3] * g);
        const uint4 va = make_uint4(pack2d(v0, v1), pack2d(v2, v3), 0u, 0u);
        st.o[dv] = mfma16d(va, pb[dv >> 1], st.o[dv]);
    }
}

template <int NW, int G>
__global__ __launch_bounds__(64 * NW, 2) void i2t0_t2i_v2_kernel(FuseArgs2 a) {
    typedef FuseOff2<G, 2> Off;
    constexpr int ABL = 0;
    constexpr int NTH = 64 * NW, NT = 256 / NW;
    __shared__ __attribute__((aligned(16))) unsigned char lds[AttnOff2::LDS > 8 * MERGE_FLOATS * 4 ? AttnOff2::LDS : 8 * MERGE_FLOATS * 4];
    const int tid = threadIdx.x, lane = tid & 63, w = __builtin_amdgcn_readfirstlane(tid >> 6), fr = lane & 15, fg = lane >> 4;
    const WaveConst wc = wave_const(fr, fg, a.Nt);
    const int voff = lane * 16, tvoff = lane * 16, vvoff = lane * 64;
    const rsrc_t rsrc = make_rsrc(a.src, T * C * 2), rq0 = make_rsrc(a.q0, T * CI * 2), rtab = make_rsrc(a.tabk, T * CI * 2),
                 rtv = make_rsrc(a.tabv, T * CI * 2);
    const unsigned char* const L = lds + lane * 16;
    if (tid < 128) ((float*)(lds + AttnOff2::GDT))[tid] = a.gd[tid];
    const float* const colc = (const float*)(lds + AttnOff2::COLC) + fr;
    const float* const gdl = (const float*)(lds + AttnOff2::GDT) + fr;
    Ring<G, 2> ring;
    for (int p = (int)blockIdx.x; p < a.P; p += (int)gridDim.x) {
        __syncthreads();
        {
            const uint4* s0 = (const uint4*)(a.oper0 + (long)p * (OPER_BYTES / 2));
            const uint4* s1 = (const uint4*)((const unsigned char*)a.aoper + (long)p * AOPER2_STRIDE);
            const uint4* s2 = (const uint4*)((const unsigned char*)a.mf + (long)p * MF_BYTES);
            for (int i = tid; i < KT_BYTES / 16; i += NTH) ((uint4*)(lds + AttnOff2::KT0))[i] = s0[KT_OFF / 16 + i];
            for (int i = tid; i < VF_BYTES / 16; i += NTH) ((uint4*)(lds + AttnOff2::VF0))[i] = s0[VF_OFF / 16 + i];
            for (int i = tid; i < AOPER2_BYTES / 16; i += NTH) ((uint4*)(lds + AttnOff2::QD2))[i] = s1[i];
            for (int i = tid; i < MF_BYTES / 16; i += NTH) ((uint4*)(lds + AttnOff2::MF2))[i] = s2[i];
            for (int i = tid; i < 16; i += NTH) ((uint4*)(lds + AttnOff2::COLC))[i] = s1[AOPER2_BYTES / 16 + i];
        }
        __syncthreads();
        AttnState st;
#pragma unroll
        for (int h = 0; h < 8; ++h) st.o[h] = f32x4_t{0.f, 0.f, 0.f, 0.f};
#pragma unroll
        for (int ct = 0; ct < 4; ++ct) { st.m[ct] = NEG_BIG; st.l[ct] = 0.f; }
        uint4 b[8], qi[4], tk[4], tv[4];
#define F2_LOAD0(tile_)                                                                            \
        do {                                                                                       \
            const int so_ = (tile_) * (16 * C * 2), to_ = (tile_) * (16 * CI * 2);                 \
            _Pragma("unroll") for (int s_ = 0; s_ < 8; ++s_) b[s_] = buf_load16(rsrc, voff, so_ + s_ * FRAG);    \
            _Pragma("unroll") for (int s_ = 0; s_ < 4; ++s_) qi[s_] = buf_load16(rq0, tvoff, to_ + s_ * FRAG);   \
        } while (0)
#define F2_LOAD1(tile_)                                                                            \
        do {                                                                                       \
            const int to_ = (tile_) * (16 * CI * 2);                                               \
            _Pragma("unroll") for (int s_ = 0; s_ < 4; ++s_) tk[s_] = buf_load16(rtab, tvoff, to_ + s_ * FRAG);  \
        } while (0)
#define F2_LOAD2(tile_)                                                                            \
        do {                                                                                       \
            const int to_ = (tile_) * (16 * CI * 2);                                               \
            _Pragma("unroll") for (int s_ = 0; s_ < 4; ++s_) tv[s_] = buf_load16(rtv, vvoff, to_ + s_ * 16);     \
        } while (0)
        F2_LOAD0(w);
        ring_fill<G, Off>(ring, L, 0);
        for (int n = 0; n < NT; ++n) {
            asm volatile("" ::: "memory");
            const int nx = w + NW * (n + 1 < NT ? n + 1 : NT - 1), cur = w + NW * n;
            uint4 y1[8], pk0[2];
            float stat[2];
            i2t_block_r<G, Off, 0, false, 0, false>(ring, L, nullptr, a.eps, b, qi, wc, y1, [&]() { F2_LOAD1(cur); }, pk0, stat);
            t2i_block_v2<G, Off, 40>(ring, L, y1, tk, tv, pk0, stat[0], stat[1], colc, gdl, st, [&]() { F2_LOAD2(cur); }, [&]() { F2_LOAD0(nx); });
#pragma unroll
            for (int i = Off::USED; i < Off::N; ++i) RING_STEP(i);
        }
#undef F2_LOAD0
#undef F2_LOAD1
#undef F2_LOAD2
#pragma unroll
        for (int ct = 0; ct < 4; ++ct) { st.l[ct] += __shfl_xor(st.l[ct], 16); st.l[ct] += __shfl_xor(st.l[ct], 32); }
        __syncthreads();
        float* mg = (float*)lds + w * MERGE_FLOATS;
        if (fg == 0) {
#pragma unroll
            for (int ct = 0; ct < 4; ++ct) { mg[ct * 16 + fr] = st.m[ct]; mg[64 + ct * 16 + fr] = st.l[ct]; }
        }
#pragma unroll
        for (int h = 0; h < 8; ++h)
            if ((fr >> 3) == (h & 1))
                *(float4*)(mg + 128 + (h * 8 + (fr & 7)) * 16 + fg * 4) = make_float4(st.o[h][0], st.o[h][1], st.o[h][2], st.o[h][3]);
        __syncthreads();
        for (int idx = tid; idx < 512; idx += NTH) {
            const int col = idx >> 3, d0 = (idx & 7) * 2, h = col >> 3, t = col & 7;
            const float* g0 = (const float*)lds;
            float mx = NEG_BIG;
#pragma unroll
            for (int ww = 0; ww < NW; ++ww) mx = fmaxf(mx, g0[ww * MERGE_FLOATS + col]);
            float lt = 0.f, o0 = 0.f, o1 = 0.f;
#pragma unroll
            for (int ww = 0; ww < NW; ++ww) {
                const float* gw = g0 + ww * MERGE_FLOATS;
                const float sc = __builtin_amdgcn_exp2f(gw[col] - mx);
                lt = fmaf(sc, gw[64 + col], lt);
                o0 = fmaf(sc, gw[128 + col * 16 + d0], o0); o1 = fmaf(sc, gw[128 + col * 16 + d0 + 1], o1);
            }
            if (t < a.Nt) {
                const float inv = 1.f / lt;
                *(uint32_t*)(a.out + ((long)p * a.Nt + t) * CI + h * 16 + d0) =
                    pack2d(fmaf(o0, inv, a.bwv[h * 16 + d0]), fmaf(o1, inv, a.bwv[h * 16 + d0 + 1]));
            }
        }
    }
}

__global__ __launch_bounds__(128) void tables2_small_kernel(const u16* __restrict__ wv, const float* __restrict__ bv,
                                                            const u16* __restrict__ wk, const float* __restrict__ gam,
                                                            const float* __restrict__ bet, const u16* __restrict__ wo0,
                                                            const float* __restrict__ bo0, unsigned char* __restrict__ t2,
                                                            long wvg_off) {
    __shared__ float wg[C], wr[C], kr[C];
    const int d = blockIdx.x, e = threadIdx.x;
    for (int c = e; c < C; c += 128) { wr[c] = d2f(wv[d * C + c]); wg[c] = wr[c] * gam[c]; kr[c] = d2f(wk[d * C + c]); }
    __syncthreads();
    float acc = 0.f;
    for (int c = 0; c < C; ++c) acc = fmaf(wg[c], d2f(wo0[c * CI + e]), acc);
    ((float*)(t2 + T2_WOWV))[d * 128 + e] = acc;
    for (int c = e; c < C; c += 128) ((u16*)(t2 + wvg_off))[d * C + c] = f2d(wg[c]);
    if (e < 4) {
        float v = 0.f;
        for (int c = 0; c < C; ++c) v += e == 0 ? wg[c] * bo0[c] : e == 1 ? wg[c] : e == 2 ? wr[c] * bet[c] : kr[c] * bet[c];
        if (e == 2) v += bv[d];
        ((float*)(t2 + (e == 0 ? T2_CD : e == 1 ? T2_GD : e == 2 ? T2_BWV : T2_KB)))[d] = v;
    }
}
__global__ __launch_bounds__(256) void tabv_relayout_kernel(const u16* __restrict__ rm, u16* __restrict__ tabv) {
    const int id = blockIdx.x * 256 + threadIdx.x;
    const int dv = id & 7, lane = (id >> 3) & 63, tile = id >> 9;
    const int row0 = tile * 16 + (lane >> 4) * 4, d = dv * 16 + (lane & 15);
    uint2 pk;
    pk.x = (uint32_t)rm[(long)row0 * CI + d] | ((uint32_t)rm[(long)(row0 + 1) * CI + d] << 16);
    pk.y = (uint32_t)rm[(long)(row0 + 2) * CI + d] | ((uint32_t)rm[(long)(row0 + 3) * CI + d] << 16);
    ((uint2*)tabv)[id] = pk;
}

__global__ __launch_bounds__(256) void fold_values_kernel(const u16* __restrict__ vtok0, int Nt, const unsigned char* __restrict__ t2,
                                                          u16* __restrict__ mf) {
    __shared__ float vv[8][CI];
    const int p = blockIdx.x, tid = threadIdx.x;
    for (int i = tid; i < 8 * CI; i += 256) {
        const int t = i >> 7, dd = i & (CI - 1);
        vv[t][dd] = t < Nt ? d2f(vtok0[((long)p * Nt + t) * CI + dd]) : 0.f;
    }
    __syncthreads();
    const int d = tid & 127, hh = tid >> 7;
    const float* wowv = (const float*)(t2 + T2_WOWV) + d * 128;
    const float cd8 = ((const float*)(t2 + T2_CD))[d] * 0.125f;
    u16* dst = mf + (long)p * (MF_BYTES / 2);
    for (int h = hh * 4; h < hh * 4 + 4; ++h) {
        float wv_[16];
#pragma unroll
        for (int e = 0; e < 16; ++e) wv_[e] = wowv[h * 16 + e];
        uint32_t pk[4];
#pragma unroll
        for (int t2_ = 0; t2_ < 4; ++t2_) {
            float a0 = 0.f, a1 = 0.f;
#pragma unroll
            for (int e = 0; e < 16; ++e) { a0 = fmaf(wv_[e], vv[2 * t2_][h * 16 + e], a0); a1 = fmaf(wv_[e], vv[2 * t2_ + 1][h * 16 + e], a1); }
            pk[t2_] = pack2d(2 * t2_ < Nt ? a0 + cd8 : 0.f, 2 * t2_ + 1 < Nt ? a1 + cd8 : 0.f);
        }
        const int a2 = h >> 2, fg = h & 3, dv = d >> 4, fr = d & 15;
        *(uint4*)(dst + (((a2 * 8 + dv) * 64 + fg * 16 + fr) * 8)) = make_uint4(pk[0], pk[1], pk[2], pk[3]);
    }
}

__global__ __launch_bounds__(256) void fold_attnfrag2_kernel(const u16* __restrict__ qtok, const u16* __restrict__ wk,
// ... 178 lines not shown
        msam_set_error("msam_i2t0_t2i_fused: null argument");
        return 1;
    }
    if (Nt < 1 || Nt > 8) { msam_set_error("msam_i2t0_t2i_fused: 1 <= Nt <= 8 tokens per prompt"); return 1; }
    if (workspace_bytes < msam_i2t0_t2i_workspace_bytes(P)) { msam_set_error("msam_i2t0_t2i_fused: workspace too small"); return 1; }
    hipStream_t s = (hipStream_t)stream;
    u16* wvfrag = (u16*)workspace;
    u16* aoper = wvfrag + WV_BYTES / 2;
    hipLaunchKernelGGL(wv_frag_kernel, dim3(128 * 32 / 256), dim3(256), 0, s, (const u16*)wv, wvfrag);
    if (int e = msam_check_launch("wv_frag")) return e;
    hipLaunchKernelGGL(fold_attnfrag_kernel, dim3(P), dim3(256), 0, s, (const u16*)qtok, (const u16*)wk, Nt, aoper);
    if (int e = msam_check_launch("fold_attnfrag")) return e;
    FuseArgs a{};
    a.src = (const u16*)src; a.q0 = (const u16*)q0; a.oper0 = (const u16*)operands0; a.ln0_w = ln0_w; a.ln0_b = ln0_b; a.eps = ln_eps;
    a.aoper = aoper; a.wvfrag = wvfrag; a.tabk = (const u16*)tabk; a.bv = bv; a.Nt = Nt; a.P = P; a.out = (u16*)out; a.tmask = g_tune_chain_tmask;
    const int cus = cu_count(), grid = P < cus ? P : cus;
    const double flops = (double)P * (T / 16) * 164.0 * 16384.0;
    msam_profile_mark2(stream, 1, flops, 0.0, 6);
    switch (g_tune_chain_variant) {
        case 1: hipLaunchKernelGGL((i2t0_t2i_ring_kernel<4, 8>), dim3(grid), dim3(256), 0, s, a); break;
        case 2: hipLaunchKernelGGL((i2t0_t2i_ring_kernel<4, 16>), dim3(grid), dim3(256), 0, s, a); break;
        case 3: hipLaunchKernelGGL((i2t0_t2i_ring_kernel<8, 4>), dim3(grid), dim3(512), 0, s, a); break;
        case 4: hipLaunchKernelGGL((i2t0_t2i_ring_kernel<8, 4, 0, 3, true>), dim3(grid), dim3(512), 0, s, a); break;
        case 5: hipLaunchKernelGGL((i2t0_t2i_ring_kernel<8, 4, 0, 2, true>), dim3(grid), dim3(512), 0, s, a); break;
        case 6: case 9: hipLaunchKernelGGL((i2t0_t2i_ring_kernel<8, 4, 0, 2, false, true>), dim3(grid), dim3(512), 0, s, a); break;
        case 7: hipLaunchKernelGGL((i2t0_t2i_ring_kernel<8, 4, 0, 3, false, true>), dim3(grid), dim3(512), 0, s, a); break;
        case 8: hipLaunchKernelGGL((i2t0_t2i_ring_kernel<8, 4, 0, 3, true, true>), dim3(grid), dim3(512), 0, s, a); break;
#define ABL_CASE(m_) case 100 + m_: hipLaunchKernelGGL((i2t0_t2i_ring_kernel<8, 4, m_>), dim3(grid), dim3(512), 0, s, a); break;
        ABL_CASE(1) ABL_CASE(2) ABL_CASE(4) ABL_CASE(8) ABL_CASE(16) ABL_CASE(32) ABL_CASE(64) ABL_CASE(27) ABL_CASE(31) ABL_CASE(127)
#undef ABL_CASE
        default: hipLaunchKernelGGL(i2t0_t2i_kernel, dim3(grid), dim3(NTHR8), 0, s, a);
    }
    msam_profile_mark2(stream, 0, flops, 0.0, 6);
    return msam_check_launch("i2t0_t2i");
}

extern "C" int64_t msam_chain_tables2_bytes(void) { return T2_BYTES; }
extern "C" int msam_chain_prepare_tables2(const void* src, const void* wv, const float* bv, const void* wk, const float* ln0_w,
                                          const float* ln0_b, const void* wo0, const float* bo0, void* tables2, void* stream) {
    if (!src || !wv || !bv || !wk || !ln0_w || !ln0_b || !wo0 || !bo0 || !tables2) { msam_set_error("msam_chain_prepare_tables2: null argument"); return 1; }
    hipStream_t s = (hipStream_t)stream;
    hipLaunchKernelGGL(tables2_small_kernel, dim3(128), dim3(128), 0, s, (const u16*)wv, bv, (const u16*)wk, ln0_w, ln0_b,
                       (const u16*)wo0, bo0, (unsigned char*)tables2, T2_WVG);
    if (int e = msam_check_launch("tables2_small")) return e;
    msam_gemm_t g{};
    g.A = src; g.lda = C; g.W = (unsigned char*)tables2 + T2_WVG; g.ldw = C; g.M = T; g.N = CI; g.K = C;
    g.out = (unsigned char*)tables2 + T2_TABV_RM; g.out_dtype = MSAM_D16; g.ldc = CI; g.a_dtype = MSAM_D16 == MSAM_F16 ? MSAM_F16 : 0;
    if (int e = msam_gemm_bf16(&g, stream)) return e;
    hipLaunchKernelGGL(tabv_relayout_kernel, dim3(T / 16 * 64 * 8 / 256), dim3(256), 0, s, (const u16*)((unsigned char*)tables2 + T2_TABV_RM),
                       (u16*)((unsigned char*)tables2 + T2_TABV));
    return msam_check_launch("tabv_relayout");
}
extern "C" int64_t msam_chain_const2_bytes(void) { return T2_TABV + (long)CI * C * 2; }
extern "C" int msam_chain_prepare_const2(const void* wv, const float* bv, const void* wk, const float* ln0_w, const float* ln0_b,
                                         const void* wo0, const float* bo0, void* const2, void* stream) {
    if (!wv || !bv || !wk || !ln0_w || !ln0_b || !wo0 || !bo0 || !const2) { msam_set_error("msam_chain_prepare_const2: null argument"); return 1; }
    hipLaunchKernelGGL(tables2_small_kernel, dim3(128), dim3(128), 0, (hipStream_t)stream, (const u16*)wv, bv, (const u16*)wk, ln0_w,
                       ln0_b, (const u16*)wo0, bo0, (unsigned char*)const2, T2_TABV);
    return msam_check_launch("tables2_small(const)");
}
extern "C" int msam_chain_prepare_tables2_c(const void* src, const void* const2, void* tables2, void* stream) {
    if (!src || !const2 || !tables2) { msam_set_error("msam_chain_prepare_tables2_c: null argument"); return 1; }
    hipStream_t s = (hipStream_t)stream;
    if (hipMemcpyAsync(tables2, const2, (size_t)T2_TABV, hipMemcpyDeviceToDevice, s) != hipSuccess) {
        msam_set_error("msam_chain_prepare_tables2_c: device copy failed");
        return 2;
    }
    msam_gemm_t g{};
    g.A = src; g.lda = C; g.W = (const unsigned char*)const2 + T2_TABV; g.ldw = C; g.M = T; g.N = CI; g.K = C;
    g.out = (unsigned char*)tables2 + T2_TABV_RM; g.out_dtype = MSAM_D16; g.ldc = CI; g.a_dtype = MSAM_D16 == MSAM_F16 ? MSAM_F16 : 0;
    if (int e = msam_gemm_bf16(&g, stream)) return e;
    hipLaunchKernelGGL(tabv_relayout_kernel, dim3(T / 16 * 64 * 8 / 256), dim3(256), 0, s, (const u16*)((unsigned char*)tables2 + T2_TABV_RM),
                       (u16*)((unsigned char*)tables2 + T2_TABV));
    return msam_check_launch("tabv_relayout");
}
extern "C" int64_t msam_t2i_fold_values_bytes(int32_t P) { return (int64_t)P * MF_BYTES; }
extern "C" int msam_t2i_fold_values(const void* vtok0, int32_t P, int32_t Nt, const void* tables2, void* mf, void* stream) {
    if (!vtok0 || !tables2 || !mf || P <= 0 || Nt < 1 || Nt > 8) { msam_set_error("msam_t2i_fold_values: bad arguments"); return 1; }
    hipLaunchKernelGGL(fold_values_kernel, dim3(P), dim3(256), 0, (hipStream_t)stream, (const u16*)vtok0, Nt, (const unsigned char*)tables2,
                       (u16*)mf);
    return msam_check_launch("fold_values");
}
extern "C" int64_t msam_i2t0_t2i_v2_workspace_bytes(int32_t P) { return (int64_t)P * AOPER2_STRIDE; }
extern "C" int msam_i2t0_t2i_fused_v2(const void* tables, const void* tables2, const void* operands0, const void* mf, const float* ln0_w,
                                      float ln_eps, const void* qtok, int32_t P, int32_t Nt, const void* wk, void* out,
                                      void* workspace, int64_t workspace_bytes, void* stream) {
    if (!tables || !tables2 || !operands0 || !mf || !ln0_w || !qtok || !wk || !out || !workspace || P <= 0) {
        msam_set_error("msam_i2t0_t2i_fused_v2: null argument");
        return 1;
    }
    if (Nt < 1 || Nt > 8) { msam_set_error("msam_i2t0_t2i_fused_v2: 1 <= Nt <= 8 tokens per prompt"); return 1; }
    if (workspace_bytes < msam_i2t0_t2i_v2_workspace_bytes(P)) { msam_set_error("msam_i2t0_t2i_fused_v2: workspace too small"); return 1; }
    hipStream_t s = (hipStream_t)stream;
    const unsigned char* t2 = (const unsigned char*)tables2;
    hipLaunchKernelGGL(fold_attnfrag2_kernel, dim3(P), dim3(256), 0, s, (const u16*)qtok, (const u16*)wk, ln0_w, t2, Nt,
                       (unsigned char*)workspace);
    if (int e = msam_check_launch("fold_attnfrag2")) return e;
    const u16* src = (const u16*)tables;
    FuseArgs2 a{};
    a.src = src; a.q0 = src + (long)T * C; a.tabk = a.q0 + (long)T * CI;
    a.tabv = (const u16*)(t2 + T2_TABV); a.gd = (const float*)(t2 + T2_GD); a.bwv = (const float*)(t2 + T2_BWV);
    a.oper0 = (const u16*)operands0; a.aoper = (const u16*)workspace; a.mf = (const u16*)mf; a.eps = ln_eps; a.Nt = Nt; a.P = P;
    a.out = (u16*)out;
    const int cus = cu_count(), grid = P < cus ? P : cus;
    const double flops = (double)P * (T / 16) * 116.0 * 16384.0;
    msam_profile_mark2(stream, 1, flops, 0.0, 6);
    hipLaunchKernelGGL((i2t0_t2i_v2_kernel<8, 4>), dim3(grid), dim3(512), 0, s, a);
    msam_profile_mark2(stream, 0, flops, 0.0, 6);
    return msam_check_launch("i2t0_t2i_v2");
}

extern "C" int msam_i2t01_fused(const void* tables, const void* operands0, const float* ln0_w, const float* ln0_b,
                                const void* operands1, const float* ln1_w, const float* ln1_b, float ln_eps,
                                int32_t P, int32_t Nt, void* out, void* stream) {
    const u16* src = (const u16*)tables;
    const u16* q0 = src ? src + (long)T * C : nullptr;
    const u16* tabq1 = src ? q0 + 2L * T * CI : nullptr;
    if (!src || !operands0 || !ln0_w || !ln0_b || !operands1 || !ln1_w || !ln1_b || !out || P <= 0) {
        msam_set_error("msam_i2t01_fused: null argument");
        return 1;
    }
    if (Nt < 1 || Nt > 8) { msam_set_error("msam_i2t01_fused: 1 <= Nt <= 8 tokens per prompt"); return 1; }
    ChainArgs a{};
    a.src = (const u16*)src; a.q0 = (const u16*)q0; a.oper0 = (const u16*)operands0; a.ln0_w = ln0_w; a.ln0_b = ln0_b;
    a.oper1 = (const u16*)operands1; a.tabq1 = (const u16*)tabq1; a.ln1_w = ln1_w; a.ln1_b = ln1_b; a.eps = ln_eps;
    a.Nt = Nt; a.P = P; a.out = (u16*)out;
    const int cus = cu_count(), grid = P < cus ? P : cus;
    const double flops = (double)P * (T / 16) * 144.0 * 16384.0;
    const double bytes = (double)P * T * C * 2;
    msam_profile_mark2(stream, 1, flops, bytes, 7);
    switch (g_tune_chain_variant) {
        case 1: hipLaunchKernelGGL((i2t01_ring_kernel<4, 8>), dim3(grid), dim3(256), 0, (hipStream_t)stream, a); break;
        case 2: hipLaunchKernelGGL((i2t01_ring_kernel<4, 16>), dim3(grid), dim3(256), 0, (hipStream_t)stream, a); break;
        case 3: case 5: hipLaunchKernelGGL((i2t01_ring_kernel<8, 4>), dim3(grid), dim3(512), 0, (hipStream_t)stream, a); break;
        case 4: hipLaunchKernelGGL((i2t01_ring_kernel<8, 4, 3>), dim3(grid), dim3(512), 0, (hipStream_t)stream, a); break;
        case 6: case 9: hipLaunchKernelGGL((i2t01_ring_kernel<8, 4, 2, true>), dim3(grid), dim3(512), 0, (hipStream_t)stream, a); break;
        case 7: case 8: hipLaunchKernelGGL((i2t01_ring_kernel<8, 4, 3, true>), dim3(grid), dim3(512), 0, (hipStream_t)stream, a); break;
        default: hipLaunchKernelGGL(i2t01_kernel, dim3(grid), dim3(NTHR8), 0, (hipStream_t)stream, a);
    }
    msam_profile_mark2(stream, 0, flops, bytes, 7);
    return msam_check_launch("i2t01");
}
```

### micro_sam_amd/csrc/decoder.hip

```cpp
#include <stdlib.h>
#include "common.h"
#include "../../include/msam_hip.h"

void msam_set_error(const char* msg);
int msam_check_launch(const char* what);

namespace {

constexpr int T = 4096;
constexpr int C = 256;
constexpr int CI = 128;
constexpr float NEG_BIG = -1.0e30f;
constexpr float TWO_PI = 6.283185307179586f;


MSAM_DEVINL void pe_encode(const float* __restrict__ G, float cx, float cy, int j, float& s, float& c) {
    const float x = 2.f * cx - 1.f, y = 2.f * cy - 1.f;
    const float v = TWO_PI * (x * G[j] + y * G[128 + j]);
    s = sinf(v); c = cosf(v);
}

__global__ __launch_bounds__(256) void dense_pe_kernel(const float* __restrict__ G, float* __restrict__ pos_f32,
                                                       u16* __restrict__ pos_bf16) {
    const int idx = blockIdx.x * 256 + threadIdx.x;
// ... 465 lines not shown
    float* pos_f32; u16* pos_bf16; float* pe_k[3]; float* pe_q[2]; u16* wkv[3]; float* bkv[3];
    u16* tab_k[3];
    u16* tab_q[2];
    void* chain2;
};
constexpr long CONST2_BYTES = 128L * 128 * 4 + 4 * 512 + (long)CI * C * 2;
constexpr long CONST_BYTES = (long)T * C * 4 + (long)T * C * 2 + 5L * T * CI * 4 + 3L * C * C * 2 + 3L * C * 4 + 5L * T * CI * 2 + CONST2_BYTES;

Consts carve_consts(void* base) {
    Consts c; char* p = (char*)base;
    c.pos_f32 = (float*)p; p += (long)T * C * 4;
    c.pos_bf16 = (u16*)p; p += (long)T * C * 2;
    for (int i = 0; i < 3; ++i) { c.pe_k[i] = (float*)p; p += (long)T * CI * 4; }
    for (int i = 0; i < 2; ++i) { c.pe_q[i] = (float*)p; p += (long)T * CI * 4; }
    for (int i = 0; i < 3; ++i) { c.wkv[i] = (u16*)p; p += (long)C * C * 2; }
    for (int i = 0; i < 3; ++i) { c.bkv[i] = (float*)p; p += (long)C * 4; }
    for (int i = 0; i < 3; ++i) { c.tab_k[i] = (u16*)p; p += (long)T * CI * 2; }
    for (int i = 0; i < 2; ++i) { c.tab_q[i] = (u16*)p; p += (long)T * CI * 2; }
    c.chain2 = p;
    return c;
}

struct ImageState { float* src_f32; u16* src_bf16; u16* k0; u16* vT0; u16* q0; };
constexpr long IMAGE_BYTES = (long)T * C * 4 + (long)T * C * 2 + 3L * T * CI * 2;

ImageState carve_image(void* base) {
    ImageState s; char* p = (char*)base;
    s.src_f32 = (float*)p; p += (long)T * C * 4;
    s.src_bf16 = (u16*)p; p += (long)T * C * 2;
    s.k0 = (u16*)p; p += (long)T * CI * 2;
    s.vT0 = (u16*)p; p += (long)T * CI * 2;
    s.q0 = (u16*)p; p += (long)T * CI * 2;
    return s;
}

inline long align256(long x) { return (x + 255) & ~255L; }

}

extern "C" int64_t msam_decoder_const_bytes(void) { return CONST_BYTES; }
extern "C" int msam_decoder_dtype(void) { return MSAM_D16; }
extern "C" int64_t msam_decoder_image_bytes(void) { return IMAGE_BYTES; }

extern "C" int msam_decoder_prepare_const(const msam_decoder_t* dec, void* consts, void* stream) {
    if (!dec || !consts) { msam_set_error("msam_decoder_prepare_const: null argument"); return 1; }
    Ctx cx{(hipStream_t)stream, dec->use_glds};
    Consts c = carve_consts(consts);
    hipLaunchKernelGGL(dense_pe_kernel, dim3(T * 128 / 256), dim3(256), 0, cx.s, dec->pe_gauss, c.pos_f32, c.pos_bf16);
    if (int e = msam_check_launch("dense_pe")) return e;
    const msam_attn_w_t* t2i[3] = {&dec->layer[0].t2i, &dec->layer[1].t2i, &dec->final_attn};
    for (int i = 0; i < 3; ++i) {
        hipMemcpyAsync(c.wkv[i], t2i[i]->k_w, (size_t)CI * C * 2, hipMemcpyDeviceToDevice, cx.s);
        hipMemcpyAsync(c.wkv[i] + (long)CI * C, t2i[i]->v_w, (size_t)CI * C * 2, hipMemcpyDeviceToDevice, cx.s);
        hipMemcpyAsync(c.bkv[i], t2i[i]->k_b, CI * 4, hipMemcpyDeviceToDevice, cx.s);
        hipMemcpyAsync(c.bkv[i] + CI, t2i[i]->v_b, CI * 4, hipMemcpyDeviceToDevice, cx.s);
        if (int e = gemm(cx, c.pos_bf16, C, t2i[i]->k_w, T, CI, C, nullptr, c.pe_k[i], MSAM_F32, CI)) return e;
        if (int e = gemm(cx, c.pos_bf16, C, t2i[i]->k_w, T, CI, C, t2i[i]->k_b, c.tab_k[i], MSAM_D16, CI)) return e;
    }
    for (int i = 0; i < 2; ++i) {
        if (int e = gemm(cx, c.pos_bf16, C, dec->layer[i].i2t.q_w, T, CI, C, nullptr, c.pe_q[i], MSAM_F32, CI)) return e;
        if (int e = gemm(cx, c.pos_bf16, C, dec->layer[i].i2t.q_w, T, CI, C, dec->layer[i].i2t.q_b, c.tab_q[i], MSAM_D16, CI))
            return e;
    }
    if (msam_chain_const2_bytes() != CONST2_BYTES) { msam_set_error("msam_decoder_prepare_const: const2 size mismatch"); return 2; }
    return msam_chain_prepare_const2(dec->layer[1].t2i.v_w, dec->layer[1].t2i.v_b, dec->layer[1].t2i.k_w, dec->layer[0].n4_w,
                                     dec->layer[0].n4_b, dec->layer[0].i2t.o_w, dec->layer[0].i2t.o_b, c.chain2, stream);
}

extern "C" int msam_decoder_prepare_image(const msam_decoder_t* dec, const void* consts, const float* embedding,
                                          void* image_state, void* workspace, int64_t workspace_bytes, void* stream) {
    (void)workspace; (void)workspace_bytes;
    if (!dec || !consts || !embedding || !image_state) { msam_set_error("msam_decoder_prepare_image: null argument"); return 1; }
    Ctx cx{(hipStream_t)stream, dec->use_glds};
    Consts c = carve_consts((void*)consts);
    ImageState im = carve_image(image_state);
    hipLaunchKernelGGL(src_prepare_kernel, dim3(T / 32, C / 32), dim3(256), 0, cx.s, embedding, dec->no_mask, im.src_f32,
                       im.src_bf16);
    if (int e = msam_check_launch("src_prepare")) return e;
    if (int e = wsgemm_kv(cx, im.src_bf16, c.wkv[0], c.bkv[0], c.pe_k[0], T, im.k0, im.vT0)) return e;
    return gemm(cx, im.src_bf16, C, dec->layer[0].i2t.q_w, T, CI, C, dec->layer[0].i2t.q_b, im.q0, MSAM_D16, CI, 0,
                nullptr, 0, 0, 0, c.pe_q[0], CI);
}

extern int g_tune_dec_chain, g_tune_dec_chain_min_p, g_tune_chain_variant;
int g_tune_tok_fuse = 0;
int g_tune_mlp_split_fused = 1;
namespace {
struct Work {
    float *qpe, *queries, *tmp; u16 *a, *b, *qs, *ks, *vs, *attn_tok, *mlp_h;
    u16 *keys, *kimg, *vT, *qimg, *attn_img, *up1; float* pre;
    u16 *hh0, *hh1; float *hyper, *iou_full;
};
long work_bytes(int P, int Nt) {
    const long M = (long)P * Nt, R = (long)P * T;
    long b = 0;
    b += 3 * align256(M * C * 4);
    b += 6 * align256(M * C * 2);
    b += align256(M * 2048 * 2);
    b += align256(R * C * 2);
    b += 4 * align256(R * CI * 2);
    b += align256(R * C * 2);
    b += align256(R * C * 4);
    b += 2 * align256(5L * P * C * 2);
    b += align256((long)P * 4 * 128 * 4) + align256((long)P * 128 * 4);
    return b;
}
Work carve_work(void* base, int P, int Nt) {
    const long M = (long)P * Nt, R = (long)P * T;
    Work w; char* p = (char*)base;
    auto take = [&](long bytes) { char* r = p; p += align256(bytes); return r; };
    w.qpe = (float*)take(M * C * 4); w.queries = (float*)take(M * C * 4); w.tmp = (float*)take(M * C * 4);
    w.a = (u16*)take(M * C * 2); w.b = (u16*)take(M * C * 2); w.qs = (u16*)take(M * C * 2); w.ks = (u16*)take(M * C * 2);
    w.vs = (u16*)take(M * C * 2); w.attn_tok = (u16*)take(M * C * 2);
    w.mlp_h = (u16*)take(M * 2048 * 2);
    w.keys = (u16*)take(R * C * 2);
    w.kimg = (u16*)take(R * CI * 2); w.vT = (u16*)take(R * CI * 2); w.qimg = (u16*)take(R * CI * 2);
    w.attn_img = (u16*)take(R * CI * 2);
    w.up1 = (u16*)take(R * C * 2);
    w.pre = (float*)take(R * C * 4);
    w.hh0 = (u16*)take(5L * P * C * 2); w.hh1 = (u16*)take(5L * P * C * 2);
    w.hyper = (float*)take((long)P * 4 * 128 * 4); w.iou_full = (float*)take((long)P * 128 * 4);
    return w;
}

int t2i_stream(const Ctx& cx, const Work& w, const Consts& c, int idx, const msam_attn_w_t& aw, int P, int Nt, bool blocked = false) {
    const long R = (long)P * T;
    if (Nt <= 8) {
        const int64_t avail = (int64_t)((char*)w.up1 - (char*)w.kimg);
        return msam_t2i_fold_attention(w.keys, blocked ? 2 : 0, w.qs, P, Nt, aw.k_w, c.tab_k[idx], aw.v_w, aw.v_b, w.attn_tok, w.kimg,
                                       avail, cx.s);
    }
    if (int e = wsgemm_kv(cx, w.keys, c.wkv[idx], c.bkv[idx], c.pe_k[idx], (int)R, w.kimg, w.vT)) return e;
    hipLaunchKernelGGL(t2i_attn_kernel, dim3(P * 8), dim3(256), 0, cx.s, w.qs, w.kimg, w.vT, 0, Nt, w.attn_tok);
    return msam_check_launch("t2i_attn");
}

__global__ void gather_iou_kernel(const float* __restrict__ iou_full, int P, int c0, int nc, float* __restrict__ iou) {
    const int i = blockIdx.x * 256 + threadIdx.x;
    if (i < P * nc) iou[i] = iou_full[(long)(i / nc) * 128 + c0 + (i % nc)];
}
}

extern "C" int64_t msam_decoder_workspace_bytes(int32_t P) { return work_bytes(P, 16); }

extern "C" int msam_decoder_forward(const msam_decoder_t* dec, const void* consts, const void* image_state,
                                    const float* points, const int32_t* labels, int32_t Np, const float* boxes, int32_t P,
                                    int32_t multimask, float* low_res, float* iou, void* workspace, int64_t workspace_bytes,
                                    void* stream) {
    return msam_decoder_forward_masks(dec, nullptr, consts, image_state, points, labels, Np, boxes, nullptr, P, multimask,
                                      low_res, iou, workspace, workspace_bytes, stream);
}

namespace {
int decoder_run(const msam_decoder_t* dec, const msam_mask_prompt_t* mask_w, const void* consts,
                const void* image_state, const float* points, const int32_t* labels, int32_t Np,
                const float* boxes, const float* mask_input, const float* sparse, int32_t Ns, const float* dense,
                const float* embedding, int32_t P, int32_t multimask,
                float* low_res, float* iou, void* workspace, int64_t workspace_bytes, void* stream);
}

extern "C" int msam_decoder_forward_masks(const msam_decoder_t* dec, const msam_mask_prompt_t* mask_w, const void* consts,
                                          const void* image_state, const float* points, const int32_t* labels, int32_t Np,
                                          const float* boxes, const float* mask_input, int32_t P, int32_t multimask,
                                          float* low_res, float* iou, void* workspace, int64_t workspace_bytes, void* stream) {
    return decoder_run(dec, mask_w, consts, image_state, points, labels, Np, boxes, mask_input, nullptr, 0, nullptr, nullptr, P,
                       multimask, low_res, iou, workspace, workspace_bytes, stream);
}

extern "C" int msam_decoder_forward_embeddings(const msam_decoder_t* dec, const void* consts, const void* image_state,
                                               const float* sparse, int32_t Ns, const float* dense, const float* embedding,
                                               int32_t P, int32_t multimask, float* low_res, float* iou, void* workspace,
                                               int64_t workspace_bytes, void* stream) {
    if (!sparse && Ns != 0) { msam_set_error("msam_decoder_forward_embeddings: Ns > 0 needs the sparse embeddings"); return 1; }
    if (Ns < 0 || Ns > 11) { msam_set_error("msam_decoder_forward_embeddings: 0 .. 11 sparse tokens per prompt"); return 1; }
    if (dense && !embedding) { msam_set_error("msam_decoder_forward_embeddings: a dense embedding needs the image embedding"); return 1; }
    return decoder_run(dec, nullptr, consts, image_state, nullptr, nullptr, 0, nullptr, nullptr, sparse ? sparse : (const float*)consts,
                       Ns, dense, embedding, P, multimask, low_res, iou, workspace, workspace_bytes, stream);
}

extern "C" int msam_prompt_encode(const msam_decoder_t* dec, const msam_mask_prompt_t* mask_w, const float* points,
                                  const int32_t* labels, int32_t Np, const float* boxes, const float* mask_input, int32_t P,
                                  float* sparse, float* dense, void* stream) {
    if (!dec || P <= 0) { msam_set_error("msam_prompt_encode: null argument"); return 1; }
    if (!points) Np = 0;
    const int Ns = Np + (boxes ? 2 : (Np > 0 ? 1 : 0));
    if (Ns > 0) {
        if (!sparse) { msam_set_error("msam_prompt_encode: null sparse output"); return 1; }
        hipLaunchKernelGGL(sparse_embed_kernel, dim3(P), dim3(256), 0, (hipStream_t)stream, dec->pe_gauss, dec->point_embed,
                           dec->not_a_point, points, labels, Np, boxes, P, Ns, sparse);
        if (int e = msam_check_launch("sparse_embed")) return e;
    }
    if (mask_input) {
        if (!mask_w || !dense) { msam_set_error("msam_prompt_encode: mask prompts need the mask_downscaling weights and a dense output"); return 1; }
        hipLaunchKernelGGL(mask_src_kernel, dim3(64, P), dim3(256), 0, (hipStream_t)stream, mask_input, *mask_w, (const float*)nullptr,
                           dec->no_mask, (u16*)nullptr, dense);
        if (int e = msam_check_launch("mask_dense")) return e;
    }
    return 0;
}

namespace {
int decoder_run(const msam_decoder_t* dec, const msam_mask_prompt_t* mask_w, const void* consts,
                const void* image_state, const float* points, const int32_t* labels, int32_t Np,
                const float* boxes, const float* mask_input, const float* sparse, int32_t Ns, const float* dense,
                const float* embedding, int32_t P, int32_t multimask,
                float* low_res, float* iou, void* workspace, int64_t workspace_bytes, void* stream) {
    if (!dec || !consts || !image_state || !low_res || !iou || !workspace || P <= 0) {
        msam_set_error("msam_decoder_forward: null argument");
        return 1;
    }
    if (!sparse && (!points || Np <= 0) && !boxes && !mask_input && !dense) {
        msam_set_error("msam_decoder_forward: need points, boxes and / or a mask prompt");
        return 1;
    }
    if (mask_input && !mask_w) { msam_set_error("msam_decoder_forward: mask prompts need the mask_downscaling weights"); return 1; }
    const bool own_src = mask_input != nullptr || dense != nullptr;
    if (!points) Np = 0;
    const int Nt = sparse ? 5 + Ns : 5 + Np + (boxes ? 2 : (Np > 0 ? 1 : 0));
    if (Nt > 16) { msam_set_error("msam_decoder_forward: at most 16 tokens per prompt (<= 10 points)"); return 1; }
    if (workspace_bytes < work_bytes(P, Nt)) { msam_set_error("msam_decoder_forward: workspace too small"); return 1; }
    Ctx cx{(hipStream_t)stream, dec->use_glds};
    Consts c = carve_consts((void*)consts);
    ImageState im = carve_image((void*)image_state);
    Work w = carve_work(workspace, P, Nt);
    const int M = P * Nt;
    const long R = (long)P * T;
    const long n4 = (long)M * C / 4;
    int e;
#define CHECK(x) do { if ((e = (x))) return e; } while (0)
#define ADD_CAST(a_, b_, out_) do { hipLaunchKernelGGL(add_cast_kernel, dim3(grid_for(n4)), dim3(256), 0, cx.s, a_, b_, out_, n4); \
                                     CHECK(msam_check_launch("add_cast")); } while (0)
#define ADD_CAST2(a_, b_, outa_, outb_) do { hipLaunchKernelGGL(add_cast2_kernel, dim3(grid_for(n4)), dim3(256), 0, cx.s, a_, b_, outa_, \
                                                                 outb_, n4); CHECK(msam_check_launch("add_cast2")); } while (0)
#define LN(x_, w_, b_, rows_, out_, dt_) CHECK(msam_layernorm(x_, w_, b_, 1e-5f, rows_, C, out_, dt_, 0, 0, cx.s))

    if (dense) {
        hipLaunchKernelGGL(dense_src_kernel, dim3(T / 32, C / 32, P), dim3(256), 0, cx.s, embedding, dense, w.keys);
        CHECK(msam_check_launch("dense_src"));
    } else if (own_src) {
        hipLaunchKernelGGL(mask_src_kernel, dim3(64, P), dim3(256), 0, cx.s, mask_input, *mask_w, im.src_f32, dec->no_mask, w.keys,
                           (float*)nullptr);
        CHECK(msam_check_launch("mask_src"));
    }
    if (sparse) {
        hipLaunchKernelGGL(tokens_from_sparse_kernel, dim3(P), dim3(256), 0, cx.s, dec->out_tokens, sparse, Ns, P, Nt, w.qpe,
                           w.queries, w.a);
        CHECK(msam_check_launch("tokens_from_sparse"));
    } else {
        hipLaunchKernelGGL(prompt_tokens_kernel, dim3(P), dim3(256), 0, cx.s, dec->pe_gauss, dec->point_embed, dec->not_a_point,
                           dec->out_tokens, points, labels, Np, boxes, P, Nt, w.qpe, w.queries, w.a);
        CHECK(msam_check_launch("prompt_tokens"));
    }

    const char* dbg = getenv("MSAM_DEBUG_DEC_LAYERS");
    const int nlayers = dbg ? atoi(dbg) : 2;
    const bool chain = g_tune_dec_chain && !own_src && !dbg && Nt <= 8 && P >= g_tune_dec_chain_min_p;
    const bool fuse_tok = g_tune_tok_fuse != 0 && !dbg;
    void* const oper0 = w.qimg; void* const oper1 = w.attn_img;
    void* const tables = (char*)w.vT + (int64_t)R * CI * 2 - msam_chain_tables_bytes();
    if (chain) CHECK(msam_chain_prepare_tables(im.src_bf16, im.q0, c.tab_k[1], c.tab_q[1], tables, cx.s));
    const bool chain2 = chain && g_tune_chain_variant == 9;
    void* const tables2 = (char*)tables - msam_chain_tables2_bytes();
    void* const mfrag = (char*)oper0 + msam_i2t_fold_operand_bytes(P);
    if (chain2) CHECK(msam_chain_prepare_tables2_c(im.src_bf16, c.chain2, tables2, cx.s));
    for (int li = 0; li < nlayers && li < 2; ++li) {
        const msam_twoway_layer_t& L = dec->layer[li];
        const u16* sv = w.a;
        if (li > 0) {
            if (!fuse_tok) ADD_CAST2(w.queries, w.qpe, w.a, w.b);
            sv = w.b;
        }
        {
            const msam_gemm_t qkv[3] = {mk_gemm(w.a, C, L.self_attn.q_w, M, C, C, L.self_attn.q_b, w.qs, MSAM_D16, C),
                                        mk_gemm(w.a, C, L.self_attn.k_w, M, C, C, L.self_attn.k_b, w.ks, MSAM_D16, C),
                                        mk_gemm(sv, C, L.self_attn.v_w, M, C, C, L.self_attn.v_b, w.vs, MSAM_D16, C)};
            CHECK(msam_gemm_group_bf16(qkv, 3, cx.s));
        }
        hipLaunchKernelGGL(token_self_attn_kernel, dim3(P), dim3(128), 0, cx.s, w.qs, w.ks, w.vs, Nt, w.attn_tok);
        CHECK(msam_check_launch("token_self_attn"));
        if (fuse_tok) {
            CHECK(gemm_ln_tok(cx, w.attn_tok, C, L.self_attn.o_w, M, C, L.self_attn.o_b, li == 0 ? nullptr : w.queries, L.n1_w, L.n1_b,
                              w.queries, w.qpe, w.a, nullptr));
        } else {
        CHECK(gemm(cx, w.attn_tok, C, L.self_attn.o_w, M, C, C, L.self_attn.o_b, w.tmp, MSAM_F32, C, 0,
                   li == 0 ? nullptr : w.queries, li == 0 ? 0 : MSAM_F32, C));
        LN(w.tmp, L.n1_w, L.n1_b, M, w.queries, MSAM_F32);
        ADD_CAST(w.queries, w.qpe, w.a);
        }
        CHECK(gemm(cx, w.a, C, L.t2i.q_w, M, CI, C, L.t2i.q_b, w.qs, MSAM_D16, CI));
        if (li == 0 && !own_src) {
            if (Nt <= 8)
                hipLaunchKernelGGL(t2i_shared4_kernel, dim3(((P + 3) / 4) * 8), dim3(256), 0, cx.s, w.qs, im.k0, im.vT0, P, Nt,
                                   w.attn_tok);
            else
                hipLaunchKernelGGL(t2i_attn_kernel, dim3(P * 8), dim3(256), 0, cx.s, w.qs, im.k0, im.vT0, 1, Nt, w.attn_tok);
            CHECK(msam_check_launch("t2i_attn"));
        } else if (chain) {
            const msam_twoway_layer_t& L0 = dec->layer[0];
            const int64_t avail = (int64_t)R * CI * 2 - msam_chain_tables_bytes() - msam_chain_tables2_bytes();
            if (chain2)
                CHECK(msam_i2t0_t2i_fused_v2(tables, tables2, oper0, mfrag, L0.n4_w, 1e-5f, w.qs, P, Nt, L.t2i.k_w, w.attn_tok, w.vT,
                                             avail, cx.s));
            else
                CHECK(msam_i2t0_t2i_fused(tables, oper0, L0.n4_w, L0.n4_b, 1e-5f, w.qs, P, Nt, L.t2i.k_w, L.t2i.v_w, L.t2i.v_b,
                                          w.attn_tok, w.vT, avail, cx.s));
        } else {
            CHECK(t2i_stream(cx, w, c, li, L.t2i, P, Nt));
        }
        if (fuse_tok) {
            CHECK(gemm_ln_tok(cx, w.attn_tok, CI, L.t2i.o_w, M, CI, L.t2i.o_b, w.queries, L.n2_w, L.n2_b, w.queries, nullptr, w.a, nullptr));
        } else {
        CHECK(gemm(cx, w.attn_tok, CI, L.t2i.o_w, M, C, CI, L.t2i.o_b, w.tmp, MSAM_F32, C, 0, w.queries, MSAM_F32, C));
        LN(w.tmp, L.n2_w, L.n2_b, M, w.queries, MSAM_F32);
        if (!(L.mlp1_ws != nullptr && L.mlp2_ws != nullptr)) ADD_CAST(w.queries, nullptr, w.a);
        }
        const bool mlp_split = L.mlp1_ws != nullptr && L.mlp2_ws != nullptr;
        const void* mlp_h = w.mlp_h; const void* mlp2_w = L.mlp2_w; int mlp2_k = 2048;
        if (mlp_split) {
            u16* a3 = (u16*)w.pre;
            float* h32 = (float*)((char*)a3 + align256((long)M * 3 * C * 2));
            u16* h3 = (u16*)((char*)h32 + align256((long)M * 2048 * 4));
            CHECK(msam_cast_f32_split16(w.queries, MSAM_D16, a3, M, C, cx.s));
            if (g_tune_mlp_split_fused) {
                msam_gemm_t g1 = mk_gemm(a3, 3 * C, L.mlp1_ws, M, 2048, 3 * C, L.mlp1_b, h3, MSAM_D16, 3 * 2048, MSAM_ACT_RELU);
                g1.out_mode = 3;
                CHECK(msam_gemm_bf16(&g1, cx.s));
            } else {
                CHECK(gemm(cx, a3, 3 * C, L.mlp1_ws, M, 2048, 3 * C, L.mlp1_b, h32, MSAM_F32, 2048, MSAM_ACT_RELU));
                CHECK(msam_cast_f32_split16(h32, MSAM_D16, h3, M, 2048, cx.s));
            }
            mlp_h = h3; mlp2_w = L.mlp2_ws; mlp2_k = 3 * 2048;
        } else {
        CHECK(gemm(cx, w.a, C, L.mlp1_w, M, 2048, C, L.mlp1_b, w.mlp_h, MSAM_D16, 2048, MSAM_ACT_RELU));
        }
        if (fuse_tok) {
            CHECK(gemm_ln_tok(cx, mlp_h, mlp2_k, mlp2_w, M, mlp2_k, L.mlp2_b, w.queries, L.n3_w, L.n3_b, w.queries, w.qpe, w.a, w.b));
        } else {
        CHECK(gemm(cx, mlp_h, mlp2_k, mlp2_w, M, C, mlp2_k, L.mlp2_b, w.tmp, MSAM_F32, C, 0, w.queries, MSAM_F32, C));
        LN(w.tmp, L.n3_w, L.n3_b, M, w.queries, MSAM_F32);
        ADD_CAST2(w.queries, w.qpe, w.a, w.b);
        }
        {
            const msam_gemm_t kv[2] = {mk_gemm(w.a, C, L.i2t.k_w, M, CI, C, L.i2t.k_b, w.ks, MSAM_D16, CI),
                                       mk_gemm(w.b, C, L.i2t.v_w, M, CI, C, L.i2t.v_b, w.vs, MSAM_D16, CI)};
            CHECK(msam_gemm_group_bf16(kv, 2, cx.s));
        }
        if (chain) {
            if (li == 0 && chain2)
                CHECK(msam_i2t_fold_operands_values(w.ks, w.vs, P, Nt, L.i2t.q_w, L.i2t.o_w, L.i2t.o_b, 0, tables2, oper0, mfrag, cx.s));
            else
                CHECK(msam_i2t_fold_operands(w.ks, w.vs, P, Nt, L.i2t.q_w, L.i2t.o_w, L.i2t.o_b, li, li == 0 ? oper0 : oper1, cx.s));
            if (li == 1) {
                const msam_twoway_layer_t& L0 = dec->layer[0];
                CHECK(msam_i2t01_fused(tables, oper0, L0.n4_w, L0.n4_b, oper1, L.n4_w, L.n4_b, 1e-5f, P, Nt, w.keys, cx.s));
            }
        } else if (Nt <= 8) {
            const bool shared = li == 0 && !own_src;
            CHECK(msam_i2t_fold_layer(shared ? (const void*)im.src_bf16 : (const void*)w.keys, shared, w.ks, w.vs, P, Nt,
                                      L.i2t.q_w, c.tab_q[li], L.i2t.o_w, L.i2t.o_b, L.n4_w, L.n4_b, 1e-5f, w.keys, w.qimg,
                                      (int64_t)((char*)w.up1 - (char*)w.qimg), cx.s));
        } else {
            msam_image_layer_t g{};
            g.wo = L.i2t.o_w; g.bo = L.i2t.o_b; g.ln_w = L.n4_w; g.ln_b = L.n4_b; g.ln_eps = 1e-5f;
            g.ktok = w.ks; g.vtok = w.vs; g.Nt = Nt; g.out = w.keys; g.rows = (int)R;
            if (li == 0 && !own_src) { g.xin = im.src_bf16; g.q_shared = im.q0; }
            else { g.xin = w.keys; g.wq = L.i2t.q_w; g.bq = L.i2t.q_b; g.peq = c.pe_q[li]; }
            CHECK(msam_decoder_image_layer(&g, cx.s));
        }
    }
    if (dbg) return 0;
    if (!fuse_tok) ADD_CAST(w.queries, w.qpe, w.a);
    CHECK(gemm(cx, w.a, C, dec->final_attn.q_w, M, CI, C, dec->final_attn.q_b, w.qs, MSAM_D16, CI));
    CHECK(t2i_stream(cx, w, c, 2, dec->final_attn, P, Nt, chain));
    if (fuse_tok) {
        CHECK(gemm_ln_tok(cx, w.attn_tok, CI, dec->final_attn.o_w, M, CI, dec->final_attn.o_b, w.queries, dec->nf_w, dec->nf_b, w.queries,
                          nullptr, w.a, nullptr));
    } else {
    CHECK(gemm(cx, w.attn_tok, CI, dec->final_attn.o_w, M, C, CI, dec->final_attn.o_b, w.tmp, MSAM_F32, C, 0, w.queries,
               MSAM_F32, C));
    LN(w.tmp, dec->nf_w, dec->nf_b, M, w.queries, MSAM_F32);

    ADD_CAST(w.queries, nullptr, w.a);
    }
    {
        msam_gemm_t h[5];
        const long PC = (long)P * C;
        for (int i = 0; i < 5; ++i) {
            const void* wt = i == 0 ? dec->iou_w[0] : dec->hyp_w[i - 1][0];
            const float* bs = i == 0 ? dec->iou_b[0] : dec->hyp_b[i - 1][0];
            h[i] = mk_gemm(w.a + (long)i * C, (long)Nt * C, wt, P, C, C, bs, w.hh0 + i * PC, MSAM_D16, C, MSAM_ACT_RELU);
        }
        CHECK(msam_gemm_group_bf16(h, 5, cx.s));
        for (int i = 0; i < 5; ++i) {
            const void* wt = i == 0 ? dec->iou_w[1] : dec->hyp_w[i - 1][1];
            const float* bs = i == 0 ? dec->iou_b[1] : dec->hyp_b[i - 1][1];
            h[i] = mk_gemm(w.hh0 + i * PC, C, wt, P, C, C, bs, w.hh1 + i * PC, MSAM_D16, C, MSAM_ACT_RELU);
        }
        CHECK(msam_gemm_group_bf16(h, 5, cx.s));
        h[0] = mk_gemm(w.hh1, C, dec->iou_w[2], P, 128, C, dec->iou_b[2], w.iou_full, MSAM_F32, 128);
        for (int i = 1; i < 5; ++i)
            h[i] = mk_gemm(w.hh1 + i * PC, C, dec->hyp_w[i - 1][2], P, 128, C, dec->hyp_b[i - 1][2], w.hyper + (long)(i - 1) * 128,
                           MSAM_F32, 4 * 128);
        CHECK(msam_gemm_group_bf16(h, 5, cx.s));
    }
    const int mask0 = multimask ? 1 : 0, nmask = multimask ? 3 : 1;
    hipLaunchKernelGGL(gather_iou_kernel, dim3((P * nmask + 255) / 256), dim3(256), 0, cx.s, w.iou_full, P, mask0, nmask, iou);
    CHECK(msam_check_launch("gather_iou"));

    CHECK(msam_upscale_fused_out(w.keys, (chain ? 1 : 0) | (dec->up1_centred ? 2 : 0), P, dec->up1_w, dec->up1_b, dec->up_ln_w, dec->up_ln_b, 1e-6f, dec->up2_w,
                                 dec->up2_b, w.hyper, 128, mask0, nmask, low_res, dec->low_res_dtype == MSAM_F16 ? MSAM_F16 : MSAM_F32,
                                 cx.s));
#undef CHECK
#undef ADD_CAST
#undef ADD_CAST2
#undef LN
    return 0;
}
}
```

### micro_sam_amd/ops.py

```python
from __future__ import annotations

import ctypes as C
from typing import Any, Dict, List, Optional, Tuple

import numpy as np
import torch

from . import _lib
from ._lib import ACT_GELU, ACT_NONE, ACT_RELU, BF16, F16, F32


_CODE16 = {torch.float32: F32, torch.bfloat16: BF16, torch.float16: F16}
_F32, _I32, _I64, _U8 = torch.float32, torch.int32, torch.int64, torch.uint8
_BITS = (torch.int32, torch.uint32)


def _code(name: str, dtype: torch.dtype) -> int:
    try:
        return _CODE16[dtype]
    except KeyError:
        raise TypeError(f"micro_sam_amd: {name} must be float32, bfloat16 or float16, got {dtype}") from None


def _home(name: str, t) -> torch.device:
# ... 893 lines not shown
    lib = _lib.load()
    t2 = torch.empty((int(lib.msam_chain_tables2_bytes()),), dtype=torch.uint8, device=src.device)
    _lib.check(lib.msam_chain_prepare_tables2(src.data_ptr(), wv.data_ptr(), bv.data_ptr(), wk.data_ptr(), ln0_w.data_ptr(),
                                              ln0_b.data_ptr(), wo0.data_ptr(), bo0.data_ptr(), t2.data_ptr(), _lib.stream_ptr()),
               "msam_chain_prepare_tables2")
    return t2


def chain_prepare_tables2_cached(src, wv, bv, wk, ln0_w, ln0_b, wo0, bo0):
    _chain2_operands(src, wv, bv, wk, ln0_w, ln0_b, wo0, bo0)
    lib = _lib.load()
    c2 = torch.empty((int(lib.msam_chain_const2_bytes()),), dtype=torch.uint8, device=src.device)
    _lib.check(lib.msam_chain_prepare_const2(wv.data_ptr(), bv.data_ptr(), wk.data_ptr(), ln0_w.data_ptr(), ln0_b.data_ptr(),
                                             wo0.data_ptr(), bo0.data_ptr(), c2.data_ptr(), _lib.stream_ptr()), "msam_chain_prepare_const2")
    t2 = torch.empty((int(lib.msam_chain_tables2_bytes()),), dtype=torch.uint8, device=src.device)
    _lib.check(lib.msam_chain_prepare_tables2_c(src.data_ptr(), c2.data_ptr(), t2.data_ptr(), _lib.stream_ptr()),
               "msam_chain_prepare_tables2_c")
    return t2, c2


def t2i_fold_values(vtok0, tables2):
    dev = _home("vtok0", vtok0)
    lib = _lib.load()
    _t("vtok0", vtok0, _lib.decoder_dtype(), (None, None, 128), dev)
    _blob("tables2", tables2, int(lib.msam_chain_tables2_bytes()), dev)
    P, Nt = vtok0.shape[0], vtok0.shape[1]
    mf = torch.empty((int(lib.msam_t2i_fold_values_bytes(P)),), dtype=torch.uint8, device=vtok0.device)
    _lib.check(lib.msam_t2i_fold_values(vtok0.data_ptr(), P, Nt, tables2.data_ptr(), mf.data_ptr(), _lib.stream_ptr()),
               "msam_t2i_fold_values")
    return mf


def i2t_fold_operands_values(ktok, vtok, wq, wo, bo, tables2, *, with_kfold: bool = False):
    dev = _home("ktok", ktok)
    lib = _lib.load()
    P, Nt = _fold_tokens(ktok, vtok, dev)
    _fold_weights(wq, wo, bo, dev)
    _blob("tables2", tables2, int(lib.msam_chain_tables2_bytes()), dev)
    oper = torch.empty((int(lib.msam_i2t_fold_operand_bytes(P)),), dtype=torch.uint8, device=ktok.device)
    mf = torch.empty((int(lib.msam_t2i_fold_values_bytes(P)),), dtype=torch.uint8, device=ktok.device)
    _lib.check(lib.msam_i2t_fold_operands_values(ktok.data_ptr(), vtok.data_ptr(), P, Nt, wq.data_ptr(), wo.data_ptr(), bo.data_ptr(),
                                                 int(with_kfold), tables2.data_ptr(), oper.data_ptr(), mf.data_ptr(),
                                                 _lib.stream_ptr()), "msam_i2t_fold_operands_values")
    return oper, mf


def i2t0_t2i_fused_v2(tables, tables2, operands0, mf, ln0_w, qtok, wk, *, ln_eps: float = 1e-5):
    dev = _home("tables", tables)
    lib = _lib.load()
    d16 = _lib.decoder_dtype()
    _t("qtok", qtok, d16, (None, None, 128), dev)
    P, Nt = qtok.shape[0], qtok.shape[1]
    _blob("tables", tables, int(lib.msam_chain_tables_bytes()), dev)
    _blob("tables2", tables2, int(lib.msam_chain_tables2_bytes()), dev)
    _blob("operands0", operands0, int(lib.msam_i2t_fold_operand_bytes(P)), dev)
    _blob("mf", mf, int(lib.msam_t2i_fold_values_bytes(P)), dev)
    _t("ln0_w", ln0_w, _F32, (256,), dev)
    _t("wk", wk, d16, (128, 256), dev)
    nbytes = int(lib.msam_i2t0_t2i_v2_workspace_bytes(P))
    work = torch.empty((nbytes,), dtype=torch.uint8, device=qtok.device)
    out = torch.empty((P, Nt, 128), dtype=d16, device=qtok.device)
    _lib.check(lib.msam_i2t0_t2i_fused_v2(tables.data_ptr(), tables2.data_ptr(), operands0.data_ptr(), mf.data_ptr(), ln0_w.data_ptr(),
                                          ln_eps, qtok.data_ptr(), P, Nt, wk.data_ptr(), out.data_ptr(), work.data_ptr(), nbytes,
                                          _lib.stream_ptr()), "msam_i2t0_t2i_fused_v2")
    return out


def i2t01_fused(tables, operands0, ln0_w, ln0_b, operands1, ln1_w, ln1_b, P: int, Nt: int, *, ln_eps: float = 1e-5):
    dev = _home("tables", tables)
    lib = _lib.load()
    _need(P > 0 and Nt > 0, f"P = {P} and Nt = {Nt} must be positive")
    _blob("tables", tables, int(lib.msam_chain_tables_bytes()), dev)
    _blob("operands0", operands0, int(lib.msam_i2t_fold_operand_bytes(P)), dev)
    _blob("operands1", operands1, int(lib.msam_i2t_fold_operand_bytes(P)), dev)
    for name, t in (("ln0_w", ln0_w), ("ln0_b", ln0_b), ("ln1_w", ln1_w), ("ln1_b", ln1_b)):
        _t(name, t, _F32, (256,), dev)
    out = torch.empty((P, 4096, 256), dtype=_lib.decoder_dtype(), device=tables.device)
    _lib.check(_lib.load().msam_i2t01_fused(tables.data_ptr(), operands0.data_ptr(), ln0_w.data_ptr(), ln0_b.data_ptr(),
                                            operands1.data_ptr(), ln1_w.data_ptr(), ln1_b.data_ptr(), ln_eps, P, Nt,
                                            out.data_ptr(), _lib.stream_ptr()), "msam_i2t01_fused")
    return out


def upscale_fused(keys, w1, b1, ln_w, ln_b, w2, b2, hyper, mask0: int, nmask: int, *, ln_eps: float = 1e-6, blocked: bool = False,
                  centred: bool = False):
    dev = _home("keys", keys)
    d16 = _lib.decoder_dtype()
    _t("keys", keys, d16, (None, 4096, 256), dev)
    P = keys.shape[0]
    _t("w1", w1, d16, (256, 256), dev)
    _t("w2", w2, d16, (128, 64), dev)
    for name, t, n in (("b1", b1, 256), ("ln_w", ln_w, 64), ("ln_b", ln_b, 64), ("b2", b2, 32)):
        _t(name, t, _F32, (n,), dev)
    _t("hyper", hyper, _F32, (P, 4, None), dev)
    _need(hyper.shape[2] >= 32 and mask0 >= 0 and nmask >= 1 and mask0 + nmask <= 4,
          f"hyper must be [P,4,>= 32] and masks [{mask0}, {mask0 + nmask}) must lie in [0, 4)")
    out = torch.empty((P, nmask, 256, 256), dtype=torch.float32, device=keys.device)
    _lib.check(_lib.load().msam_upscale_fused_layout(keys.data_ptr(), int(blocked) | (2 if centred else 0), P, w1.data_ptr(), b1.data_ptr(), ln_w.data_ptr(),
                                                     ln_b.data_ptr(), ln_eps, w2.data_ptr(), b2.data_ptr(), hyper.data_ptr(),
                                                     hyper.shape[-1], mask0, nmask, out.data_ptr(), _lib.stream_ptr()),
               "msam_upscale_fused_layout")
    return out


def upscale_centre_weights(w1_f32: torch.Tensor, b1_f32: torch.Tensor):
    w = w1_f32.float().view(4, 64, -1)
    b = b1_f32.float().view(4, 64)
    return ((w - w.mean(1, keepdim=True)).reshape(256, -1).to(_lib.decoder_dtype()).contiguous(),
            (b - b.mean(1, keepdim=True)).reshape(256).contiguous())


def uncrop_bits(bits: torch.Tensor, crop_box, height: int, width: int) -> torch.Tensor:
    _home("bits", bits)
    x0, y0, x1, y1 = (int(v) for v in crop_box)
    if bits.dtype not in _BITS:
        raise TypeError(f"micro_sam_amd: bits must be int32 / uint32 words, got {bits.dtype}")
    _need(bits.dim() == 3 and tuple(bits.shape[1:]) == ((y1 - y0 + 31) // 32, x1 - x0),
          f"bits must be [N, ceil(crop_h / 32), crop_w] of crop_box {[x0, y0, x1, y1]}, got {list(bits.shape)}")
    n = int(bits.shape[0])
    out = torch.empty((n, (height + 31) // 32, width), dtype=torch.int32, device=bits.device)
    if n == 0:
        return out
    bits = bits.contiguous()
    lib = _lib.load()
    step = 65535
    for s in range(0, n, step):
        m = min(step, n - s)
        _lib.check(lib.msam_uncrop_bits(bits[s:].data_ptr(), m, y1 - y0, x1 - x0, x0, y0, height, width, out[s:].data_ptr(),
                                        _lib.stream_ptr()), "msam_uncrop_bits")
    return out


from ._matching import label_matching
from ._labelprops import DistanceTargets, LabelProps, distance_targets, edt_squared, label_props
from ._propagate import mask_box_prompts, mask_iou_counts, mask_logits, pack_bits, paint_max
from ._embedpca import PCA_MAX_CHANNELS, PCA_MAX_COMPONENTS, PCA_MAX_UNITS, pca_moments, pca_moments_workspace_bytes, pca_project, pca_to_rgb
from ._semloss import SEMLOSS_MAX_CLASSES, SemanticLossStats, semantic_loss, semantic_loss_backward
from ._depthconv import depth_conv3
```

Before: 177.4 tiles/s.

## Hand over layer-0 i2t fragments and LN stats from fused v2 kernel to i2t01

The fused i2t0+t2i v2 kernel now writes its per-tile layer-0 attention output fragments and layernorm statistics to a handover buffer. The later i2t01 kernel reads them instead of recomputing the layer-0 image-to-token block, which skips about 8 of its 112 ring fragments and their MFMAs. This trades the recompute for extra global stores and loads of about 256 tiles per prompt, plus a larger workspace. It also adds a split-offset ring addressing path and a tunable ring depth.

New measurement: 179.4 tiles/s (median of 6 runs). 1.2% higher.

```diff
diff --git a/include/msam_hip.h b/include/msam_hip.h
--- a/include/msam_hip.h
+++ b/include/msam_hip.h
@@ -108,6 +108,13 @@
                            int64_t workspace_bytes, void* stream);
 int msam_i2t01_fused(const void* tables, const void* operands0, const float* ln0_w, const float* ln0_b, const void* operands1,
                      const float* ln1_w, const float* ln1_b, float ln_eps, int32_t P, int32_t Nt, void* out, void* stream);
+int64_t msam_chain_handover_bytes(int32_t P);
+int msam_i2t0_t2i_fused_v2_handover(const void* tables, const void* tables2, const void* operands0, const void* mf, const float* ln0_w,
+                                    float ln_eps, const void* qtok, int32_t P, int32_t Nt, const void* wk, void* out, void* workspace,
+                                    int64_t workspace_bytes, void* handover, void* stream);
+int msam_i2t01_fused_handover(const void* tables, const void* operands0, const float* ln0_w, const float* ln0_b, const void* operands1,
+                              const float* ln1_w, const float* ln1_b, float ln_eps, int32_t P, int32_t Nt, const void* handover,
+                              void* out, void* stream);
 
 int msam_upscale_fused(const void* keys, int32_t P, const void* w1, const float* b1, const float* ln_w, const float* ln_b,
                        float ln_eps, const void* w2, const float* b2, const float* hyper, int32_t hyper_ld, int32_t mask0,
diff --git a/micro_sam_amd/_lib.py b/micro_sam_amd/_lib.py
--- a/micro_sam_amd/_lib.py
+++ b/micro_sam_amd/_lib.py
@@ -169,6 +169,9 @@
     "msam_i2t_fold_operands_values": (_i32, [_vp, _vp, _i32, _i32, _vp, _vp, _vp, _i32, _vp, _vp, _vp, _vp]),
     "msam_i2t0_t2i_v2_workspace_bytes": (_i64, [_i32]),
     "msam_i2t0_t2i_fused_v2": (_i32, [_vp, _vp, _vp, _vp, _vp, _f32, _vp, _i32, _i32, _vp, _vp, _vp, _i64, _vp]),
+    "msam_chain_handover_bytes": (_i64, [_i32]),
+    "msam_i2t0_t2i_fused_v2_handover": (_i32, [_vp, _vp, _vp, _vp, _vp, _f32, _vp, _i32, _i32, _vp, _vp, _vp, _i64, _vp, _vp]),
+    "msam_i2t01_fused_handover": (_i32, [_vp, _vp, _vp, _vp, _vp, _vp, _vp, _f32, _i32, _i32, _vp, _vp, _vp]),
     "msam_chain_tables_bytes": (_i64, []),
     "msam_chain_prepare_tables": (_i32, [_vp, _vp, _vp, _vp, _vp, _vp]),
     "msam_upscale_fused_layout": (_i32, [_vp, _i32, _i32, _vp, _vp, _vp, _vp, _f32, _vp, _vp, _vp, _i32, _i32, _i32, _vp, _vp]),
diff --git a/micro_sam_amd/csrc/decfold.hip b/micro_sam_amd/csrc/decfold.hip
--- a/micro_sam_amd/csrc/decfold.hip
+++ b/micro_sam_amd/csrc/decfold.hip
@@ -700,6 +700,7 @@
 void msam_gemm_set_g3(int delay);
 void msam_gemm_set_g3_epi(int v);
 extern int g_tune_tok_fuse;
+extern int g_tune_chain_handover, g_tune_chain_handover_ring;
 extern int g_tune_mlp_split_fused;
 extern int g_tune_sgemm_bufs, g_tune_srel_mfma, g_tune_sgemm_small_below, g_tune_si2t_dbg, g_tune_si2t_late_us, g_tune_sattn_allh;
 int g_tune_dec_chain = 1, g_tune_dec_chain_min_p = 128;
@@ -710,6 +711,8 @@
     else if (k == "dec_chain") g_tune_dec_chain = value;
     else if (k == "chain_variant") g_tune_chain_variant = value;
     else if (k == "chain_tmask") g_tune_chain_tmask = value;
+    else if (k == "chain_handover") g_tune_chain_handover = value;
+    else if (k == "chain_handover_ring") g_tune_chain_handover_ring = value;
     else if (k == "up_gelu16") g_tune_up_gelu16 = value;
     else if (k == "up_ln_two_pass") g_tune_up_ln_two_pass = value;
     else if (k == "up_centred") g_tune_up_centred = value;
diff --git a/micro_sam_amd/csrc/decfold_tok.hip b/micro_sam_amd/csrc/decfold_tok.hip
--- a/micro_sam_amd/csrc/decfold_tok.hip
+++ b/micro_sam_amd/csrc/decfold_tok.hip
@@ -9,6 +9,8 @@
 int g_tune_i2t_wg_per_cu = 2;
 int g_tune_chain_tmask = 255;
 int g_tune_chain_variant = 9;
+int g_tune_chain_handover = 1;
+int g_tune_chain_handover_ring = 3;
 
 namespace {
 
@@ -268,7 +270,11 @@
     const float* ln1_w; const float* ln1_b;
     float eps; int Nt, P;
     u16* out;
+    const unsigned char* hand;
 };
+
+constexpr int HAND_STAT = 2 * FRAG, HAND_TILE = HAND_STAT + 16 * 8;
+constexpr long HAND_PROMPT = 256L * HAND_TILE;
 
 constexpr int NTHR8 = 512;
 constexpr int C_KT0 = 0, C_VF0 = C_KT0 + KT_BYTES, C_KT1 = C_VF0 + VF_BYTES, C_KF1 = C_KT1 + KT_BYTES, C_VF1 = C_KF1 + KF_BYTES,
@@ -507,13 +513,17 @@
     }
 }
 
-template <int G, int D = 2> struct Ring { uint4 buf[D][G]; };
+template <int G, int D = 2> struct Ring { uint4 buf[D][G]; int hi; };
 
 template <int G, class Off, int ABL = 0>
 MSAM_DEVINL void ring_fill(Ring<G, Off::D>& r, const unsigned char* L, int batch) {
     if (ABL & 32) return;
 #pragma unroll
-    for (int j = 0; j < G; ++j) r.buf[batch % Off::D][j] = *(const uint4*)(L + Off::off((batch * G + j) % Off::N));
+    for (int j = 0; j < G; ++j) {
+        const int o = Off::off((batch * G + j) % Off::N);
+        if (Off::SPLIT && o >= 65536) r.buf[batch % Off::D][j] = *(const uint4*)(L + r.hi + (o - 65536));
+        else r.buf[batch % Off::D][j] = *(const uint4*)(L + o);
+    }
 }
 #define RING_STEP(n_) do { if ((n_) % G == 0) { TK_FENCE(); ring_fill<G, Off, ABL>(ring, L, (n_) / G + Off::D - 1); TK_FENCE(); } } while (0)
 #define RING_AT(n_) ring.buf[((n_) / G) % Off::D][(n_) % G]
@@ -665,6 +675,7 @@
 
 template <int G, int D_ = 2> struct ChainOff {
     static constexpr int D = D_, USED = 112, N = ((USED + D * G - 1) / (D * G)) * (D * G);
+    static constexpr bool SPLIT = false;
     static __device__ constexpr int off(int n) {
         if (n < 8) return C_KT0 + ((n % 4) * 2 + n / 4) * FRAG;
         if (n < 40) return C_VF0 + (n - 8) * FRAG;
@@ -675,6 +686,7 @@
 };
 template <int G, int D_ = 2> struct FuseOff {
     static constexpr int D = D_, USED = 140, N = ((USED + D * G - 1) / (D * G)) * (D * G);
+    static constexpr bool SPLIT = false;
     static __device__ constexpr int off(int n) {
         if (n < 8) return F_KT0 + ((n % 4) * 2 + n / 4) * FRAG;
         if (n < 40) return F_VF0 + (n - 8) * FRAG;
@@ -745,6 +757,111 @@
     }
 }
 
+template <int G, int D_ = 2> struct ChainOffH {
+    static constexpr int D = D_, USED = 104, N = ((USED + D * G - 1) / (D * G)) * (D * G);
+    static constexpr bool SPLIT = true;
+    static __device__ constexpr int off(int n) {
+        if (n < 32) return C_VF0 + n * FRAG;
+        if (n < 72) { const int i = n - 32, g = i / 4, m = i % 4; return g < 8 ? C_KF1 + (m * 8 + g) * FRAG : C_KT1 + (m * 2 + (g - 8)) * FRAG; }
+        if (n < 104) return C_VF1 + (n - 72) * FRAG;
+        return C_VF0;
+    }
+};
+
+template <int G, class Off, int BASE, class F>
+MSAM_DEVINL void i2t_block_h(Ring<G, Off::D>& ring, const unsigned char* L, const float* gp, const uint4* b, const uint4* pk,
+                             const uint4& stat2, const WaveConst& wc, uint4* y, F&& consumed) {
+    constexpr int ABL = 0;
+    f32x4_t o[16];
+#pragma unroll
+    for (int ct = 0; ct < 16; ++ct) o[ct] = mfma16d(wc.sel[ct & 1], b[ct >> 1], f32x4_t{0.f, 0.f, 0.f, 0.f});
+    consumed();
+#pragma unroll
+    for (int i = 0; i < 32; ++i) {
+        const int n = BASE + i;
+        RING_STEP(n);
+        o[i % 16] = mfma16d(RING_AT(n), pk[i / 16], o[i % 16]);
+    }
+    const bool odd = (__lane_id() & 1) != 0;
+    const float rstd = __uint_as_float(odd ? stat2.z : stat2.x), nmr = __uint_as_float(odd ? stat2.w : stat2.y);
+#pragma unroll
+    for (int c2 = 0; c2 < 8; ++c2) {
+        const float4 g0 = *(const float4*)(gp + c2 * 32), g1 = *(const float4*)(gp + c2 * 32 + 4);
+        const float4 h0 = *(const float4*)(gp + C + c2 * 32), h1 = *(const float4*)(gp + C + c2 * 32 + 4);
+        const f32x4_t x0 = o[2 * c2], x1 = o[2 * c2 + 1];
+        y[c2].x = pack2d(fmaf(fmaf(x0[0], rstd, nmr), g0.x, h0.x), fmaf(fmaf(x0[1], rstd, nmr), g0.y, h0.y));
+        y[c2].y = pack2d(fmaf(fmaf(x0[2], rstd, nmr), g0.z, h0.z), fmaf(fmaf(x0[3], rstd, nmr), g0.w, h0.w));
+        y[c2].z = pack2d(fmaf(fmaf(x1[0], rstd, nmr), g1.x, h1.x), fmaf(fmaf(x1[1], rstd, nmr), g1.y, h1.y));
+        y[c2].w = pack2d(fmaf(fmaf(x1[2], rstd, nmr), g1.z, h1.z), fmaf(fmaf(x1[3], rstd, nmr), g1.w, h1.w));
+    }
+}
+
+template <int G, int D>
+__global__ __launch_bounds__(NTHR8, 2) void i2t01_hand_kernel(ChainArgs a) {
+    typedef ChainOffH<G, D> Off;
+    constexpr int ABL = 0;
+    constexpr int NW = 8, NT = 256 / NW;
+    __shared__ __attribute__((aligned(16))) unsigned char lds[C_LDS];
+    const int tid = threadIdx.x, lane = tid & 63, w = __builtin_amdgcn_readfirstlane(tid >> 6), fr = lane & 15, fg = lane >> 4;
+    float* prm = (float*)(lds + C_PRM);
+    for (int i = tid; i < 4 * C; i += NTHR8) prm[i] = i < C ? a.ln0_w[i] : i < 2 * C ? a.ln0_b[i - C] : i < 3 * C ? a.ln1_w[i - 2 * C] : a.ln1_b[i - 3 * C];
+    const WaveConst wc = wave_const(fr, fg, a.Nt);
+    const int voff = lane * 16;
+    const int soff = (fr >> 1) * 16;
+    const rsrc_t rsrc = make_rsrc(a.src, T * C * 2), rtab = make_rsrc(a.tabq1, T * CI * 2);
+    const unsigned char* const L = lds + lane * 16;
+    const float* const gp0 = prm + fg * 8;
+    const float* const gp1 = prm + 2 * C + fg * 8;
+    Ring<G, D> ring;
+    ring.hi = 65536;
+    asm volatile("" : "+v"(ring.hi));
+    for (int p = (int)blockIdx.x; p < a.P; p += (int)gridDim.x) {
+        __syncthreads();
+        {
+            int ptid = w * 64 + (voff >> 4);
+            asm volatile("" : "+v"(ptid));
+            const uint4* s0 = (const uint4*)(a.oper0 + (long)p * (OPER_BYTES / 2));
+            const uint4* s1 = (const uint4*)(a.oper1 + (long)p * (OPER_BYTES / 2));
+            for (int i = ptid; i < VF_BYTES / 16; i += NTHR8) ((uint4*)(lds + C_VF0))[i] = s0[VF_OFF / 16 + i];
+#pragma unroll 3
+            for (int i = ptid; i < OPER_BYTES / 16; i += NTHR8) ((uint4*)(lds + C_KT1))[i] = s1[i];
+        }
+        __syncthreads();
+        const rsrc_t ro = make_rsrc(a.out + (long)p * T * C, T * C * 2);
+        const rsrc_t rh = make_rsrc(a.hand + (long)p * HAND_PROMPT, (uint32_t)HAND_PROMPT);
+        uint4 b[8], pk[2], tb[4], st;
+#define CH_LOAD0(tile_)                                                                            \
+        do {                                                                                       \
+            const int so_ = (tile_) * (16 * C * 2), ho_ = (tile_) * HAND_TILE;                     \
+            _Pragma("unroll") for (int s_ = 0; s_ < 8; ++s_) b[s_] = buf_load16(rsrc, voff, so_ + s_ * FRAG);    \
+            pk[0] = buf_load16(rh, voff, ho_); pk[1] = buf_load16(rh, voff, ho_ + FRAG);           \
+            st = buf_load16(rh, soff, ho_ + HAND_STAT);                                            \
+        } while (0)
+#define CH_LOAD1(tile_)                                                                            \
+        do {                                                                                       \
+            const int to_ = (tile_) * (16 * CI * 2);                                               \
+            _Pragma("unroll") for (int s_ = 0; s_ < 4; ++s_) tb[s_] = buf_load16(rtab, voff, to_ + s_ * FRAG);   \
+        } while (0)
+        CH_LOAD0(w);
+        wait_vmem_all();
+#pragma unroll
+        for (int k = 0; k + 1 < D; ++k) ring_fill<G, Off>(ring, L, k);
+        for (int n = 0; n < NT; ++n) {
+            asm volatile("" ::: "memory");
+            const int tile = w + NW * n, nx = w + NW * (n + 1 < NT ? n + 1 : NT - 1);
+            uint4 y1[8], y2[8];
+            i2t_block_h<G, Off, 0>(ring, L, gp0, b, pk, st, wc, y1, [&]() { CH_LOAD1(tile); });
+            i2t_block_r<G, Off, 32, true>(ring, L, gp1, a.eps, y1, tb, wc, y2, [&]() { CH_LOAD0(nx); });
+#pragma unroll
+            for (int i = Off::USED; i < Off::N; ++i) RING_STEP(i);
+#pragma unroll
+            for (int c2 = 0; c2 < 8; ++c2) buf_store16(y2[c2], ro, voff, tile * (16 * C * 2) + c2 * FRAG);
+        }
+#undef CH_LOAD0
+#undef CH_LOAD1
+    }
+}
+
 template <int NW, int G, int ABL = 0, int D = 2, bool COMPACT = false, bool LATE = false>
 __global__ __launch_bounds__(64 * NW, NW == 4 ? 1 : 2) void i2t0_t2i_ring_kernel(FuseArgs a) {
     typedef FuseOff<G, D> Off;
@@ -861,8 +978,9 @@
                T2_TABV = T2_KB + 512, T2_WVG = T2_TABV + (long)T * CI * 2 ,
                T2_TABV_RM = T2_WVG + (long)CI * C * 2 , T2_BYTES = T2_TABV_RM + (long)T * CI * 2;
 
-template <int G, int D_ = 2> struct FuseOff2 {
+template <int G, int D_ = 2, bool SPLIT_ = false> struct FuseOff2 {
     static constexpr int D = D_, USED = 92, N = ((USED + D * G - 1) / (D * G)) * (D * G);
+    static constexpr bool SPLIT = SPLIT_;
     static __device__ constexpr int off(int n) {
         if (n < 8) return AttnOff2::KT0 + ((n % 4) * 2 + n / 4) * FRAG;
         if (n < 40) return AttnOff2::VF0 + (n - 8) * FRAG;
@@ -880,6 +998,7 @@
     const u16* mf;
     float eps; int Nt, P;
     u16* out;
+    unsigned char* hand;
 };
 
 template <int G, class Off, int BASE, class F0, class F>
@@ -949,9 +1068,10 @@
     }
 }
 
-template <int NW, int G>
+template <int NW, int G, int HD = 0>
 __global__ __launch_bounds__(64 * NW, 2) void i2t0_t2i_v2_kernel(FuseArgs2 a) {
-    typedef FuseOff2<G, 2> Off;
+    constexpr bool HAND = HD != 0;
+    typedef FuseOff2<G, HAND ? HD : 2, HAND> Off;
     constexpr int ABL = 0;
     constexpr int NTH = 64 * NW, NT = 256 / NW;
     __shared__ __attribute__((aligned(16))) unsigned char lds[AttnOff2::LDS > 8 * MERGE_FLOATS * 4 ? AttnOff2::LDS : 8 * MERGE_FLOATS * 4];
@@ -964,18 +1084,22 @@
     if (tid < 128) ((float*)(lds + AttnOff2::GDT))[tid] = a.gd[tid];
     const float* const colc = (const float*)(lds + AttnOff2::COLC) + fr;
     const float* const gdl = (const float*)(lds + AttnOff2::GDT) + fr;
-    Ring<G, 2> ring;
+    Ring<G, Off::D> ring;
+    ring.hi = 65536;
+    if (HAND) asm volatile("" : "+v"(ring.hi));
     for (int p = (int)blockIdx.x; p < a.P; p += (int)gridDim.x) {
         __syncthreads();
+        int ptid = tid, plane = lane;
+        if (HAND) asm volatile("" : "+v"(ptid), "+v"(plane));
         {
             const uint4* s0 = (const uint4*)(a.oper0 + (long)p * (OPER_BYTES / 2));
             const uint4* s1 = (const uint4*)((const unsigned char*)a.aoper + (long)p * AOPER2_STRIDE);
             const uint4* s2 = (const uint4*)((const unsigned char*)a.mf + (long)p * MF_BYTES);
-            for (int i = tid; i < KT_BYTES / 16; i += NTH) ((uint4*)(lds + AttnOff2::KT0))[i] = s0[KT_OFF / 16 + i];
-            for (int i = tid; i < VF_BYTES / 16; i += NTH) ((uint4*)(lds + AttnOff2::VF0))[i] = s0[VF_OFF / 16 + i];
-            for (int i = tid; i < AOPER2_BYTES / 16; i += NTH) ((uint4*)(lds + AttnOff2::QD2))[i] = s1[i];
-            for (int i = tid; i < MF_BYTES / 16; i += NTH) ((uint4*)(lds + AttnOff2::MF2))[i] = s2[i];
-            for (int i = tid; i < 16; i += NTH) ((uint4*)(lds + AttnOff2::COLC))[i] = s1[AOPER2_BYTES / 16 + i];
+            for (int i = ptid; i < KT_BYTES / 16; i += NTH) ((uint4*)(lds + AttnOff2::KT0))[i] = s0[KT_OFF / 16 + i];
+            for (int i = ptid; i < VF_BYTES / 16; i += NTH) ((uint4*)(lds + AttnOff2::VF0))[i] = s0[VF_OFF / 16 + i];
+            for (int i = ptid; i < AOPER2_BYTES / 16; i += NTH) ((uint4*)(lds + AttnOff2::QD2))[i] = s1[i];
+            for (int i = ptid; i < MF_BYTES / 16; i += NTH) ((uint4*)(lds + AttnOff2::MF2))[i] = s2[i];
+            for (int i = ptid; i < 16; i += NTH) ((uint4*)(lds + AttnOff2::COLC))[i] = s1[AOPER2_BYTES / 16 + i];
         }
         __syncthreads();
         AttnState st;
@@ -984,6 +1108,7 @@
 #pragma unroll
         for (int ct = 0; ct < 4; ++ct) { st.m[ct] = NEG_BIG; st.l[ct] = 0.f; }
         uint4 b[8], qi[4], tk[4], tv[4];
+        const rsrc_t rh = make_rsrc(HAND ? a.hand + (long)p * HAND_PROMPT : nullptr, HAND ? (uint32_t)HAND_PROMPT : 0u);
 #define F2_LOAD0(tile_)                                                                            \
         do {                                                                                       \
             const int so_ = (tile_) * (16 * C * 2), to_ = (tile_) * (16 * CI * 2);                 \
@@ -1001,14 +1126,21 @@
             _Pragma("unroll") for (int s_ = 0; s_ < 4; ++s_) tv[s_] = buf_load16(rtv, vvoff, to_ + s_ * 16);     \
         } while (0)
         F2_LOAD0(w);
-        ring_fill<G, Off>(ring, L, 0);
+#pragma unroll
+        for (int k = 0; k + 1 < Off::D; ++k) ring_fill<G, Off>(ring, L, k);
         for (int n = 0; n < NT; ++n) {
             asm volatile("" ::: "memory");
             const int nx = w + NW * (n + 1 < NT ? n + 1 : NT - 1), cur = w + NW * n;
             uint4 y1[8], pk0[2];
             float stat[2];
             i2t_block_r<G, Off, 0, false, 0, false>(ring, L, nullptr, a.eps, b, qi, wc, y1, [&]() { F2_LOAD1(cur); }, pk0, stat);
-            t2i_block_v2<G, Off, 40>(ring, L, y1, tk, tv, pk0, stat[0], stat[1], colc, gdl, st, [&]() { F2_LOAD2(cur); }, [&]() { F2_LOAD0(nx); });
+            t2i_block_v2<G, Off, 40>(ring, L, y1, tk, tv, pk0, stat[0], stat[1], colc, gdl, st, [&]() {
+                F2_LOAD2(cur);
+                if (HAND) {
+                    buf_store16(pk0[0], rh, voff, cur * HAND_TILE); buf_store16(pk0[1], rh, voff, cur * HAND_TILE + FRAG);
+                    if (fg == 0) buf_store8(make_uint2(__float_as_uint(stat[0]), __float_as_uint(stat[1])), rh, fr * 8, cur * HAND_TILE + HAND_STAT);
+                }
+            }, [&]() { F2_LOAD0(nx); });
 #pragma unroll
             for (int i = Off::USED; i < Off::N; ++i) RING_STEP(i);
         }
@@ -1019,16 +1151,17 @@
         for (int ct = 0; ct < 4; ++ct) { st.l[ct] += __shfl_xor(st.l[ct], 16); st.l[ct] += __shfl_xor(st.l[ct], 32); }
         __syncthreads();
         float* mg = (float*)lds + w * MERGE_FLOATS;
-        if (fg == 0) {
-#pragma unroll
-            for (int ct = 0; ct < 4; ++ct) { mg[ct * 16 + fr] = st.m[ct]; mg[64 + ct * 16 + fr] = st.l[ct]; }
+        const int mfr = plane & 15, mfg = plane >> 4;
+        if (mfg == 0) {
+#pragma unroll
+            for (int ct = 0; ct < 4; ++ct) { mg[ct * 16 + mfr] = st.m[ct]; mg[64 + ct * 16 + mfr] = st.l[ct]; }
         }
 #pragma unroll
         for (int h = 0; h < 8; ++h)
-            if ((fr >> 3) == (h & 1))
-                *(float4*)(mg + 128 + (h * 8 + (fr & 7)) * 16 + fg * 4) = make_float4(st.o[h][0], st.o[h][1], st.o[h][2], st.o[h][3]);
-        __syncthreads();
-        for (int idx = tid; idx < 512; idx += NTH) {
+            if ((mfr >> 3) == (h & 1))
+                *(float4*)(mg + 128 + (h * 8 + (mfr & 7)) * 16 + mfg * 4) = make_float4(st.o[h][0], st.o[h][1], st.o[h][2], st.o[h][3]);
+        __syncthreads();
+        for (int idx = ptid; idx < 512; idx += NTH) {
             const int col = idx >> 3, d0 = (idx & 7) * 2, h = col >> 3, t = col & 7;
             const float* g0 = (const float*)lds;
             float mx = NEG_BIG;
@@ -1373,9 +1506,10 @@
     return msam_check_launch("fold_values");
 }
 extern "C" int64_t msam_i2t0_t2i_v2_workspace_bytes(int32_t P) { return (int64_t)P * AOPER2_STRIDE; }
-extern "C" int msam_i2t0_t2i_fused_v2(const void* tables, const void* tables2, const void* operands0, const void* mf, const float* ln0_w,
-                                      float ln_eps, const void* qtok, int32_t P, int32_t Nt, const void* wk, void* out,
-                                      void* workspace, int64_t workspace_bytes, void* stream) {
+extern "C" int64_t msam_chain_handover_bytes(int32_t P) { return (int64_t)P * HAND_PROMPT; }
+static int i2t0_t2i_v2_launch(const void* tables, const void* tables2, const void* operands0, const void* mf, const float* ln0_w,
+                              float ln_eps, const void* qtok, int32_t P, int32_t Nt, const void* wk, void* out,
+                              void* workspace, int64_t workspace_bytes, void* handover, void* stream) {
     if (!tables || !tables2 || !operands0 || !mf || !ln0_w || !qtok || !wk || !out || !workspace || P <= 0) {
         msam_set_error("msam_i2t0_t2i_fused_v2: null argument");
         return 1;
@@ -1392,13 +1526,26 @@
     a.src = src; a.q0 = src + (long)T * C; a.tabk = a.q0 + (long)T * CI;
     a.tabv = (const u16*)(t2 + T2_TABV); a.gd = (const float*)(t2 + T2_GD); a.bwv = (const float*)(t2 + T2_BWV);
     a.oper0 = (const u16*)operands0; a.aoper = (const u16*)workspace; a.mf = (const u16*)mf; a.eps = ln_eps; a.Nt = Nt; a.P = P;
-    a.out = (u16*)out;
+    a.out = (u16*)out; a.hand = (unsigned char*)handover;
     const int cus = cu_count(), grid = P < cus ? P : cus;
     const double flops = (double)P * (T / 16) * 116.0 * 16384.0;
-    msam_profile_mark2(stream, 1, flops, 0.0, 6);
-    hipLaunchKernelGGL((i2t0_t2i_v2_kernel<8, 4>), dim3(grid), dim3(512), 0, s, a);
-    msam_profile_mark2(stream, 0, flops, 0.0, 6);
+    const double bytes = handover ? (double)P * HAND_PROMPT : 0.0;
+    msam_profile_mark2(stream, 1, flops, bytes, 6);
+    if (handover) hipLaunchKernelGGL((i2t0_t2i_v2_kernel<8, 4, 3>), dim3(grid), dim3(512), 0, s, a);
+    else hipLaunchKernelGGL((i2t0_t2i_v2_kernel<8, 4>), dim3(grid), dim3(512), 0, s, a);
+    msam_profile_mark2(stream, 0, flops, bytes, 6);
     return msam_check_launch("i2t0_t2i_v2");
+}
+extern "C" int msam_i2t0_t2i_fused_v2(const void* tables, const void* tables2, const void* operands0, const void* mf, const float* ln0_w,
+                                      float ln_eps, const void* qtok, int32_t P, int32_t Nt, const void* wk, void* out,
+                                      void* workspace, int64_t workspace_bytes, void* stream) {
+    return i2t0_t2i_v2_launch(tables, tables2, operands0, mf, ln0_w, ln_eps, qtok, P, Nt, wk, out, workspace, workspace_bytes, nullptr, stream);
+}
+extern "C" int msam_i2t0_t2i_fused_v2_handover(const void* tables, const void* tables2, const void* operands0, const void* mf,
+                                               const float* ln0_w, float ln_eps, const void* qtok, int32_t P, int32_t Nt, const void* wk,
+                                               void* out, void* workspace, int64_t workspace_bytes, void* handover, void* stream) {
+    if (!handover) { msam_set_error("msam_i2t0_t2i_fused_v2_handover: null argument"); return 1; }
+    return i2t0_t2i_v2_launch(tables, tables2, operands0, mf, ln0_w, ln_eps, qtok, P, Nt, wk, out, workspace, workspace_bytes, handover, stream);
 }
 
 extern "C" int msam_i2t01_fused(const void* tables, const void* operands0, const float* ln0_w, const float* ln0_b,
@@ -1432,3 +1579,26 @@
     msam_profile_mark2(stream, 0, flops, bytes, 7);
     return msam_check_launch("i2t01");
 }
+
+extern "C" int msam_i2t01_fused_handover(const void* tables, const void* operands0, const float* ln0_w, const float* ln0_b,
+                                         const void* operands1, const float* ln1_w, const float* ln1_b, float ln_eps,
+                                         int32_t P, int32_t Nt, const void* handover, void* out, void* stream) {
+    const u16* src = (const u16*)tables;
+    if (!src || !operands0 || !ln0_w || !ln0_b || !operands1 || !ln1_w || !ln1_b || !handover || !out || P <= 0) {
+        msam_set_error("msam_i2t01_fused_handover: null argument");
+        return 1;
+    }
+    if (Nt < 1 || Nt > 8) { msam_set_error("msam_i2t01_fused_handover: 1 <= Nt <= 8 tokens per prompt"); return 1; }
+    ChainArgs a{};
+    a.src = src; a.oper0 = (const u16*)operands0; a.ln0_w = ln0_w; a.ln0_b = ln0_b;
+    a.oper1 = (const u16*)operands1; a.tabq1 = src + (long)T * C + 2L * T * CI; a.ln1_w = ln1_w; a.ln1_b = ln1_b; a.eps = ln_eps;
+    a.Nt = Nt; a.P = P; a.out = (u16*)out; a.hand = (const unsigned char*)handover;
+    const int cus = cu_count(), grid = P < cus ? P : cus;
+    const double flops = (double)P * (T / 16) * 136.0 * 16384.0;
+    const double bytes = (double)P * T * C * 2 + (double)P * HAND_PROMPT;
+    msam_profile_mark2(stream, 1, flops, bytes, 7);
+    if (g_tune_chain_handover_ring == 2) hipLaunchKernelGGL((i2t01_hand_kernel<4, 2>), dim3(grid), dim3(NTHR8), 0, (hipStream_t)stream, a);
+    else hipLaunchKernelGGL((i2t01_hand_kernel<4, 3>), dim3(grid), dim3(NTHR8), 0, (hipStream_t)stream, a);
+    msam_profile_mark2(stream, 0, flops, bytes, 7);
+    return msam_check_launch("i2t01_handover");
+}
diff --git a/micro_sam_amd/csrc/decoder.hip b/micro_sam_amd/csrc/decoder.hip
--- a/micro_sam_amd/csrc/decoder.hip
+++ b/micro_sam_amd/csrc/decoder.hip
@@ -571,7 +571,7 @@
                 nullptr, 0, 0, 0, c.pe_q[0], CI);
 }
 
-extern int g_tune_dec_chain, g_tune_dec_chain_min_p, g_tune_chain_variant;
+extern int g_tune_dec_chain, g_tune_dec_chain_min_p, g_tune_chain_variant, g_tune_chain_handover;
 int g_tune_tok_fuse = 0;
 int g_tune_mlp_split_fused = 1;
 namespace {
@@ -579,6 +579,7 @@
     float *qpe, *queries, *tmp; u16 *a, *b, *qs, *ks, *vs, *attn_tok, *mlp_h;
     u16 *keys, *kimg, *vT, *qimg, *attn_img, *up1; float* pre;
     u16 *hh0, *hh1; float *hyper, *iou_full;
+    void* hand;
 };
 long work_bytes(int P, int Nt) {
     const long M = (long)P * Nt, R = (long)P * T;
@@ -592,6 +593,7 @@
     b += align256(R * C * 4);
     b += 2 * align256(5L * P * C * 2);
     b += align256((long)P * 4 * 128 * 4) + align256((long)P * 128 * 4);
+    b += align256(msam_chain_handover_bytes(P));
     return b;
 }
 Work carve_work(void* base, int P, int Nt) {
@@ -609,6 +611,7 @@
     w.pre = (float*)take(R * C * 4);
     w.hh0 = (u16*)take(5L * P * C * 2); w.hh1 = (u16*)take(5L * P * C * 2);
     w.hyper = (float*)take((long)P * 4 * 128 * 4); w.iou_full = (float*)take((long)P * 128 * 4);
+    w.hand = take(msam_chain_handover_bytes(P));
     return w;
 }
 
@@ -752,6 +755,7 @@
     void* const tables2 = (char*)tables - msam_chain_tables2_bytes();
     void* const mfrag = (char*)oper0 + msam_i2t_fold_operand_bytes(P);
     if (chain2) CHECK(msam_chain_prepare_tables2_c(im.src_bf16, c.chain2, tables2, cx.s));
+    const bool handover = chain2 && g_tune_chain_handover != 0;
     for (int li = 0; li < nlayers && li < 2; ++li) {
         const msam_twoway_layer_t& L = dec->layer[li];
         const u16* sv = w.a;
@@ -787,7 +791,10 @@
         } else if (chain) {
             const msam_twoway_layer_t& L0 = dec->layer[0];
             const int64_t avail = (int64_t)R * CI * 2 - msam_chain_tables_bytes() - msam_chain_tables2_bytes();
-            if (chain2)
+            if (handover)
+                CHECK(msam_i2t0_t2i_fused_v2_handover(tables, tables2, oper0, mfrag, L0.n4_w, 1e-5f, w.qs, P, Nt, L.t2i.k_w, w.attn_tok,
+                                                      w.vT, avail, w.hand, cx.s));
+            else if (chain2)
                 CHECK(msam_i2t0_t2i_fused_v2(tables, tables2, oper0, mfrag, L0.n4_w, 1e-5f, w.qs, P, Nt, L.t2i.k_w, w.attn_tok, w.vT,
                                              avail, cx.s));
             else
@@ -841,7 +848,10 @@
                 CHECK(msam_i2t_fold_operands(w.ks, w.vs, P, Nt, L.i2t.q_w, L.i2t.o_w, L.i2t.o_b, li, li == 0 ? oper0 : oper1, cx.s));
             if (li == 1) {
                 const msam_twoway_layer_t& L0 = dec->layer[0];
-                CHECK(msam_i2t01_fused(tables, oper0, L0.n4_w, L0.n4_b, oper1, L.n4_w, L.n4_b, 1e-5f, P, Nt, w.keys, cx.s));
+                if (handover)
+                    CHECK(msam_i2t01_fused_handover(tables, oper0, L0.n4_w, L0.n4_b, oper1, L.n4_w, L.n4_b, 1e-5f, P, Nt, w.hand, w.keys, cx.s));
+                else
+                    CHECK(msam_i2t01_fused(tables, oper0, L0.n4_w, L0.n4_b, oper1, L.n4_w, L.n4_b, 1e-5f, P, Nt, w.keys, cx.s));
             }
         } else if (Nt <= 8) {
             const bool shared = li == 0 && !own_src;
diff --git a/micro_sam_amd/ops.py b/micro_sam_amd/ops.py
--- a/micro_sam_amd/ops.py
+++ b/micro_sam_amd/ops.py
@@ -999,6 +999,51 @@
     return out
 
 
+def _chain_handover_buffer(P: int, device) -> torch.Tensor:
+    _need(P > 0, f"P = {P} must be positive")
+    return torch.empty((int(_lib.load().msam_chain_handover_bytes(P)),), dtype=torch.uint8, device=device)
+
+
+def _i2t0_t2i_fused_v2_handover(tables, tables2, operands0, mf, ln0_w, qtok, wk, handover, *, ln_eps: float = 1e-5):
+    dev = _home("tables", tables)
+    lib = _lib.load()
+    d16 = _lib.decoder_dtype()
+    _t("qtok", qtok, d16, (None, None, 128), dev)
+    P, Nt = qtok.shape[0], qtok.shape[1]
+    _blob("tables", tables, int(lib.msam_chain_tables_bytes()), dev)
+    _blob("tables2", tables2, int(lib.msam_chain_tables2_bytes()), dev)
+    _blob("operands0", operands0, int(lib.msam_i2t_fold_operand_bytes(P)), dev)
+    _blob("mf", mf, int(lib.msam_t2i_fold_values_bytes(P)), dev)
+    _blob("handover", handover, int(lib.msam_chain_handover_bytes(P)), dev)
+    _t("ln0_w", ln0_w, _F32, (256,), dev)
+    _t("wk", wk, d16, (128, 256), dev)
+    nbytes = int(lib.msam_i2t0_t2i_v2_workspace_bytes(P))
+    work = torch.empty((nbytes,), dtype=torch.uint8, device=qtok.device)
+    out = torch.empty((P, Nt, 128), dtype=d16, device=qtok.device)
+    _lib.check(lib.msam_i2t0_t2i_fused_v2_handover(tables.data_ptr(), tables2.data_ptr(), operands0.data_ptr(), mf.data_ptr(),
+                                                   ln0_w.data_ptr(), ln_eps, qtok.data_ptr(), P, Nt, wk.data_ptr(), out.data_ptr(),
+                                                   work.data_ptr(), nbytes, handover.data_ptr(), _lib.stream_ptr()),
+               "msam_i2t0_t2i_fused_v2_handover")
+    return out
+
+
+def _i2t01_fused_handover(tables, operands0, ln0_w, ln0_b, operands1, ln1_w, ln1_b, P: int, Nt: int, handover, *, ln_eps: float = 1e-5):
+    dev = _home("tables", tables)
+    lib = _lib.load()
+    _need(P > 0 and Nt > 0, f"P = {P} and Nt = {Nt} must be positive")
+    _blob("tables", tables, int(lib.msam_chain_tables_bytes()), dev)
+    _blob("operands0", operands0, int(lib.msam_i2t_fold_operand_bytes(P)), dev)
+    _blob("operands1", operands1, int(lib.msam_i2t_fold_operand_bytes(P)), dev)
+    _blob("handover", handover, int(lib.msam_chain_handover_bytes(P)), dev)
+    for name, t in (("ln0_w", ln0_w), ("ln0_b", ln0_b), ("ln1_w", ln1_w), ("ln1_b", ln1_b)):
+        _t(name, t, _F32, (256,), dev)
+    out = torch.empty((P, 4096, 256), dtype=_lib.decoder_dtype(), device=tables.device)
+    _lib.check(lib.msam_i2t01_fused_handover(tables.data_ptr(), operands0.data_ptr(), ln0_w.data_ptr(), ln0_b.data_ptr(),
+                                             operands1.data_ptr(), ln1_w.data_ptr(), ln1_b.data_ptr(), ln_eps, P, Nt,
+                                             handover.data_ptr(), out.data_ptr(), _lib.stream_ptr()), "msam_i2t01_fused_handover")
+    return out
+
+
 def upscale_fused(keys, w1, b1, ln_w, ln_b, w2, b2, hyper, mask0: int, nmask: int, *, ln_eps: float = 1e-6, blocked: bool = False,
                   centred: bool = False):
     dev = _home("keys", keys)
```
